# wei-zeng98/piano-a2s

Measured on AMD Instinct MI355X. Metric: training clips/sec (12 s, 5-bar), higher is better.
Workload: dtype f32

## Files before the change

### include/a2s.h

```cpp
#ifndef A2S_H
#define A2S_H
#include <stddef.h>
#include <stdint.h>
#ifdef __cplusplus
extern "C" {
#endif

#define A2S_OK 0
#define A2S_ERR_ARG (-1)
#define A2S_ERR_HIP (-2)
#define A2S_ERR_WORKSPACE (-3)

const char* a2s_last_error(void);
int a2s_version(void);
long long a2s_launch_count(void);

int a2s_gemm_f32(void* stream, int M, int N, int K, float alpha, const float* A, long sAm, long sAk,
                 const float* B, long sBk, long sBn, float beta, float* C, long ldc, const float* bias, int act,
                 int batch, long bsA, long bsB, long bsC, int splitk, float* workspace, size_t workspace_bytes);
int a2s_gemm_f32_affine(void* stream, int M, int N, int K, float alpha, const float* A, long sAm, long sAk, const float* B, long sBk,
                        long sBn, float beta, float* C, long ldc, const float* bias, int act, int batch, long bsA, long bsB, long bsC,
                        int splitk, float* workspace, size_t workspace_bytes, const float* a_scale, const float* a_shift, int a_period,
                        const float* b_scale, const float* b_shift, int b_period);
int a2s_gemm_f32_bnstats(void* stream, int M, int N, int K, const float* A, long sAm, long sAk, const float* B, long sBk, long sBn, float* C, long ldc,
                         const float* y, const float* mean, const float* invstd, const float* scale, const float* shift, int period, float* partial);
int a2s_gemm_f32_affine_scaled(void* stream, int M, int N, int K, float alpha, const float* A, long sAm, long sAk, const float* B, long sBk,
                               long sBn, float beta, float* C, long ldc, const float* bias, int act, int batch, long bsA, long bsB, long bsC,
                               int splitk, float* workspace, size_t workspace_bytes, const float* a_scale, const float* a_shift, int a_period,
                               const float* b_scale, const float* b_shift, int b_period, const float* a_absmax, const float* b_absmax);
int a2s_gemm_f32_bnstats_scaled(void* stream, int M, int N, int K, const float* A, long sAm, long sAk, const float* B, long sBk, long sBn, float* C, long ldc,
                                const float* y, const float* mean, const float* invstd, const float* scale, const float* shift, int period, float* partial,
                                const float* a_absmax, const float* b_absmax);
int a2s_linear_dgrad_bnstats(void* stream, int M, int N, int K, const float* dz, long lda, const float* Wt, float* da, long ldc, const float* y,
                             const float* mean, const float* invstd, const float* scale, const float* shift, int period, float* partial,
                             const float* dz_absmax, const float* w_absmax, float* workspace, size_t workspace_bytes, float* da_absmax_out);
int a2s_linear_fwd(void* stream, int M, int N, int K, const float* y, long lda, const float* W, float* z, long ldc, const float* scale, const float* shift,
                   int period, const float* y_absmax, const float* w_absmax, float* workspace, size_t workspace_bytes);
int a2s_linear_fwd_eligible(int M, int N, int K, int period);
int a2s_linear_wgrad(void* stream, int M, int N, int K, const float* dz, long ldz, const float* y, long lda, float* G, long ldg, const float* scale,
                     const float* shift, int period, const float* dz_absmax, const float* y_absmax, float* workspace, size_t workspace_bytes);
size_t a2s_linear_wgrad_ws_bytes(int M, int K);
int a2s_linear_wgrad_eligible(int M, int N, int K, int period);
int a2s_tallk_wgrad(void* stream, int M, int Np, int K, const float* P, long ldp, const float* A, long lda, float* G, long ldg, int transposed, float* bias,
                    const float* p_absmax, const float* a_absmax, float* workspace, size_t workspace_bytes);
size_t a2s_tallk_wgrad_ws_bytes(int M, int Np, int K);
int a2s_tallk_wgrad_eligible(int M, int Np, int K, long ldp, long lda, long ldg, int transposed);
size_t a2s_linear_dgrad_ws_bytes(int N, int K);
int a2s_linear_dgrad_blocks(int M);
int a2s_linear_dgrad_eligible(int M, int N, int K, int period);
int a2s_absmax(void* stream, const float* x, long n, float* out);
int a2s_gemm_bnstats_blocks(int M, int period);
size_t a2s_gemm_workspace_bytes(int M, int N, int batch, int splitk);
int a2s_gemm_pick_splitk(int M, int N, int K, int batch);
void a2s_gemm_debug_tile(int cfg);
int a2s_debug_set(const char* key, int value);
int a2s_debug_get(const char* key);
int a2s_env_check(void);
int a2s_persist_abort_latch(void* device_word);

int a2s_conv3x3(void* stream, const float* x, const float* w, float* y, const float* in_scale, const float* in_shift,
                float* stat_partial, int B, int T, int F, int Cin, int Cout, int flip, float* workspace);
int a2s_conv3x3_ranged(void* stream, const float* x, const float* w, float* y, const float* in_scale, const float* in_shift, const float* in_absmax,
                       float* stat_partial, float* out_absmax, int B, int T, int F, int Cin, int Cout, float* workspace);
int a2s_conv3x3_stat_blocks(int B, int T, int F, int Cin);
int a2s_conv3x3_dgrad_bnstats(void* stream, const float* dy, const float* w, float* g, const float* yl, const float* yl_mean, const float* yl_invstd,
                              const float* yl_scale, const float* yl_shift, float* stat_partial, int B, int T, int F, int Cin, int Cout,
                              float* workspace);
int a2s_bn_bwd_from_partial(void* stream, const float* g, const float* x, const float* mean, const float* invstd, const float* scale, const float* shift,
                            float* dgamma, float* dbeta, float* dx , const float* partial, int nblocks, float* c12, long rows, int C, int F);
int a2s_conv3x3_dgrad_bnstats_scaled(void* stream, const float* dy, const float* w, float* g, const float* yl, const float* yl_mean, const float* yl_invstd,
                                     const float* yl_scale, const float* yl_shift, float* stat_partial, int B, int T, int F, int Cin, int Cout,
                                     float* workspace, const float* dy_absmax);
int a2s_conv3x3_dgrad_bnstats_ranged(void* stream, const float* dy, const float* w, float* g, const float* yl, const float* yl_mean, const float* yl_invstd,
                                     const float* yl_scale, const float* yl_shift, float* stat_partial, int B, int T, int F, int Cin, int Cout,
                                     float* workspace, const float* dy_absmax, float* g_absmax_out);
int a2s_bn_bwd_from_partial_amax(void* stream, const float* g, const float* x, const float* mean, const float* invstd, const float* scale, const float* shift,
                                 float* dgamma, float* dbeta, float* dx, const float* partial, int nblocks, float* c12, long rows, int C, int F,
                                 float* dx_absmax);
size_t a2s_conv3x3_workspace_floats(int Cin);
int a2s_bn_finalize(void* stream, const float* partial, int nblocks, int C, double count, const float* gamma,
                    const float* beta, float* running_mean, float* running_var, long long* num_batches_tracked,
                    float* mean, float* invstd, float* scale, float* shift, float eps, float momentum, int training);
int a2s_bn_relu_apply(void* stream, const float* x, float* y, const float* scale, const float* shift, long n, int C, int F);
int a2s_col_stats(void* stream, const float* x, float* partial, long rows, int C, int rows_per_block);
int a2s_bn1d_relu_dropout(void* stream, const float* x, float* y, const float* scale, const float* shift,
                          const uint8_t* keep_mask, float inv_keep, long n, int C);

int a2s_gru_gates_fwd(void* stream, const float* gi, long ldgi, const float* gh, long ldgh, const float* hprev, long ldhp,
                      float* hout, long ldho, float* hout2, long ldho2, float* save, int R, int H);
int a2s_gru_seq_fwd(void* stream, const float* gi_all, long gi_bstride, long gi_tstride, const float* w_hh,
                    const float* b_hh, float* out, long out_bstride, long out_tstride, float* hbuf, float* gh,
                    float* save, float* hn, int B, int T, int H, int reverse, float* workspace, size_t workspace_bytes);

int a2s_attn_step_fwd(void* stream, const float* keys, const float* enc, const float* q, long ldq, const float* v,
                      float* ctx, long ldctx, float* ctx2, long ldctx2, float* attw, int B, int T, int H,
                      const int* n_done, int n_rows_total, float* workspace);
int a2s_attn_step_fwd_rows(void* stream, const float* keys, const float* enc, const float* q, long ldq, const float* v, float* ctx,
                           long ldctx, float* ctx2, long ldctx2, float* attw, int R, int T, int H, float* workspace, int n_clips,
                           const int* clip_order, const int* clip_rank, const int* row_until, int n_active, int step);
size_t a2s_attn_workspace_floats(int B, int T, int H);
size_t a2s_attn_workspace_floats_fused(int n_clips, int T, int H, int groups);

int a2s_log_softmax_rows(void* stream, const float* x, long ldx, float* y, long ldy, int* argmax_out, int R, int V);
int a2s_embed_rows(void* stream, const float* table, const long long* ids64, const int* ids32, long id_stride,
                   int const_id, float* out, long ldo, int col0, int R, int E, const uint8_t* keep_mask, float inv_keep);

typedef struct a2s_note_dec_args {
    const float* attn_w; const float* attn_b; const float* attn_v;
    const float* w_ih; const float* w_hh; const float* b_ih; const float* b_hh;
    const float* out_w; const float* out_b; const float* emb;
    const float* keys; const float* enc;
    float* h; float* x; float* q; float* gates; float* attw; float* o;
    float* gh; float* gi; float* logits;
    float* probs; long probs_bstride;
    const long long* gt; long gt_bstride;
    const uint8_t* tf_flags;
    const uint8_t* drop; float inv_keep;
    int* argmax_out; long am_bstride;
    int* eos_seen; long long* lengths; int* n_done;
    int* steps_exec;
    float* attn_ws;
    float* gemm_ws; size_t gemm_ws_bytes;
    int* t_base;
    const int* clip_order;
    const int* clip_rank;
    const int* row_until;
    const int* n_active;
    int n_clips;
    const int* m_active;
    const int* row_list;
    const int* n_rows_active;
    int R, T, H, E, V, steps, poll, eos_id;
    int use_graph;
    float* step_ws; size_t step_ws_floats;
    const int* tf_flags_dev;
    float* persist_ws; size_t persist_ws_bytes;
} a2s_note_dec_args;
int a2s_note_decoder_fwd(void* stream, const a2s_note_dec_args* args, int* steps_done);
int a2s_grammar_argmax_rows(void* stream, const float* x, long ldx, float* y, long ldy, const signed char* next_state, int n_states, int* row_state,
                            int* choice_out, int R, int V);
int a2s_note_decoder_fwd_grammar(void* stream, const a2s_note_dec_args* args, const signed char* next_state, int n_states, int* row_state, int* steps_done);
int a2s_grammar_launches(void);
#define A2S_BEAM_MAX 4
typedef struct a2s_beam_args {
    int K; float alpha;
    const signed char* next_state; int n_states;
    int pad_id;
    int* row_state;
    float* score; int* finished;
    int* done_count;
    int* token_hist; int* parent_hist; float* score_hist;
    float* probs_scratch;
    int* ids_out; long long* lengths_out; float* score_out;
} a2s_beam_args;
int a2s_note_decoder_fwd_beam(void* stream, const a2s_note_dec_args* args, const a2s_beam_args* beam, int* steps_done);
int a2s_beam_step(void* stream, const a2s_beam_args* beam, const float* logits, long ldl, const float* emb, float* xnext, long ldx, float* h, int h_cols,
                  float* q, int q_cols, int* n_done, int* steps_exec, int B, int V, int E, int t, int max_steps, int eos_id);
int a2s_beam_backtrack(void* stream, const a2s_beam_args* beam, float* probs, long probs_bstride, const int* steps_exec, int B, int V, int max_steps, int eos_id);
int a2s_beam_launches(void);
typedef struct a2s_align_args {
    float* attw_step;
    int* peak; float* weight; float* centroid;
    long out_stride;
    const signed char* next_state; int n_states;
    int* row_state;
} a2s_align_args;
int a2s_attn_align_rows(void* stream, const float* attw, long ldw, int R, int T, int* peak_out, float* weight_out, float* centroid_out, long out_stride);
int a2s_note_decoder_fwd_align(void* stream, const a2s_note_dec_args* args, const a2s_align_args* align, int* steps_done);
int a2s_align_launches(void);

int a2s_render_notes(void* stream, const int* programs, int rows_per_clip, int n_samples, float* wave, long wave_bstride, int B);
int a2s_render_launches(void);

int a2s_transpose_targets(void* stream, const int* new_key, const int* interval, const int* token_map, int n_rows, int V, const int* semitones,
                          const float* detune, long long* key, long long* upper, long long* lower, int bars, int U, int L, int bins_per_semitone,
                          float* eff_bins, int* counters, int B);
int a2s_shift_bins(void* stream, const float* x, float* y, const float* eff_bins, int B, int rows, int F);
int a2s_augment_launches(void);

int a2s_tempo_plan(void* stream, const float* x, int B, int rows, int F, const float* u, float R, int min_frames, int* content, int* step,
                   int* counters);
int a2s_stretch_frames(void* stream, const float* x, float* y, const int* step, int B, int rows, int F);
int a2s_tempo_launches(void);

int a2s_specaug_plan(void* stream, const float* x, int B, int rows, int F, const float* table, const unsigned* draws, int Wt, int Wf, int m,
                     int* content, int* plan, float* stats, int* counters);
int a2s_specaug_apply(void* stream, const float* x, float* y, const float* table, const int* content, const int* plan, const float* stats, int B,
                      int rows, int F);
int a2s_specaug_launches(void);

int a2s_room_ir(void* stream, const unsigned* room_seed, const int* params, int B, float* ir, long ir_bstride, int L_max);
int a2s_fir_rows(void* stream, const float* x, long x_bstride, const float* ir, long ir_bstride, const int* params, float* y, long y_bstride, int B,
                 int n_samples, int L_max);
int a2s_fir_tile_samples(void);
int a2s_fir_tap_chunk(void);
int a2s_room_launches(void);

int a2s_resample_rows(void* stream, const float* x, long x_bstride, const int* n_in, int n_in_max, int C, const float* table, int L, int M, int K, int Hh,
                      float* y, long y_bstride, int n_out_max, int B);
int a2s_resample_tile_samples(void);
int a2s_resample_launches(void);

// ... 141 lines not shown
```

### piano_a2s_amd/conv_bwd_plan.py

```python
from collections import namedtuple

CHANS = ((1, 20), (20, 20), (20, 40), (40, 40))
LIN_WGRAD_PLACES = ("before", "beside", 4, 3, 2)


class ConvBwdFlags(namedtuple("ConvBwdFlags", "fuse_bn_rows dgrad_bnstats sync_fused fuse_bn_apply fuse_bn_apply_l1 lin_wgrad_at",
                              defaults=(True, True, True, False, True, "before"))):
    """The switches of engine_bwd (module attributes there, read once per call), with their defaults.
    fuse_bn_rows: BatchNorm-backward apply inside the row-streaming weight gradient's staging waves (A2S_FUSE_BN_ROWS=0: a tensor pass of its own).
    dgrad_bnstats: the statistics of the layer below in the epilogue of the data gradient (the Linear's included).
    sync_fused: synchronised BatchNorm keeps these fused paths (one small all-reduce per layer); False: separate statistics + apply passes.
    fuse_bn_apply / fuse_bn_apply_l1: the apply inside the TILED weight gradient a2s_conv3x3_wgrad_bn (dy = scale (g' - c1 - xhat c2) formed while the
    kernel stages its dy operand), for every layer (parity-tested, slower: the extra operand pushes conv3x3_wgrad<40> from 202 to 281 registers) / for
    conv1, whose weight gradient is a kernel of its own and whose input gradient nothing else reads (one pass over (g, y) instead of two).
    lin_wgrad_at: where the Linear's weight gradient (reads y4 once, 10-11 ms, only the optimizer waits for it) is issued: "before" the data gradient on
    the main stream; "beside" it on the weight-gradient stream; 4 / 3 / 2: on that stream at the top of that layer's turn.  Step time in that order:
    454.6, 454.5, 456.9, 456.3, 463.3 ms (profiles/r06_ab_switches.txt, r06_ab_lin_wgrad_placement.txt): no placement of this launch moves the step;
    the simplest is the default."""


class LinearPlan(namedtuple("LinearPlan", "stats absmax_after dgrad wgrad_at join_side")):
    """stats: statistics source of the BatchNorm1d above the Linear (always the full form: "own" / "sync_own"); absmax_after: max |dz| by a pass of its own
    (the synchronised apply does not reduce it).  dgrad: "own" (csrc/a2s_linear.hip: partials and max |da|), "generic" (two-term GEMM tiles with the
    statistics epilogue: partials) or "gemm" (neither).  wgrad_at: see ConvBwdFlags.lin_wgrad_at; join_side: the weight gradient ran on the
    weight-gradient stream, so the main stream waits for that stream at the end of the ConvStack backward."""


class LayerPlan(namedtuple("LayerPlan", "i ci co dy_range form stats absmax_after lin_wgrad dgrad dgrad_range out_range")):
    """Layer i with channels ci -> co.
    dy_range: the layer owns a device scalar max |dy|, zeroed by the executor and reduced by the kernel that writes dy: the two-term fp16 kernels that read dy scale
    it by the matching power of two (gradients would otherwise sit in fp16's subnormal range).
    form: how BatchNorm backward and weight gradient are launched.
      "rows"  -- statistics only, then a2s_conv3x3_wgrad_bn_ranged: dy = scale (g' - c1 - xhat c2) is formed by the STAGING waves of the row-streaming
                 kernel (they wait 40-57 % of their time for the multiply waves) and written once, over g in place (every element is read and written
                 by the same thread), with its range: one pass over (g, y) less than "apply".  Needs partials and a range with the incoming gradient.
      "apply" -- the full BatchNorm backward over g in place, which writes the range (absmax_after: the synchronised one does not; a2s_absmax does),
                 then a2s_conv3x3_wgrad_ranged.
      "tiled" -- statistics only, then a2s_conv3x3_wgrad_bn, which forms dy while it stages its operand and writes it to a fresh tensor; no range.
                 Layer 1 has no data gradient, so its dy is never written: one pass over (g, y) instead of apply (read 2, write 1) + read 1.
    stats: see stats_source.  lin_wgrad: the Linear's weight gradient is issued on the weight-gradient stream before anything of this layer.
    dgrad: "bnstats" (a2s_conv3x3_dgrad_bnstats_ranged: partials for the layer below in its epilogue; dgrad_range: it is given the layer's max |dy|;
    out_range: it writes the per-channel range of what it produces), "plain" (a2s_conv3x3, flip = 1: nothing for the layer below) or "none" (layer 1)."""


def stats_source(sync_bn, stats_only, has_partial):
    if has_partial and not sync_bn:
        return "partial"
    if has_partial and stats_only:
        return "sync_partial"
    if sync_bn and stats_only:
        raise ValueError("synchronised BatchNorm backward, statistics only, without the producer's partials: not a plan")
    return "sync_own" if sync_bn else "own"


def plan_convstack_bwd(flags, sync_bn, rows, F, linear_kernels, linear_dgrad_eligible, ranged_eligible):
    if isinstance(flags.lin_wgrad_at, bool) or flags.lin_wgrad_at not in LIN_WGRAD_PLACES:
        raise ValueError(f"lin_wgrad_at = {flags.lin_wgrad_at!r}: expected one of {LIN_WGRAD_PLACES}")
    fused_ok = not sync_bn or flags.sync_fused
    stats = flags.dgrad_bnstats and fused_ok
    epilogue = stats and F >= 128 and F % 4 == 0 and rows > 64
    dgrad = ("own" if linear_kernels and linear_dgrad_eligible else "generic") if epilogue else "gemm"
    linear = LinearPlan(stats_source(sync_bn, False, False), sync_bn, dgrad, flags.lin_wgrad_at, flags.lin_wgrad_at != "before")
    partial, amax = dgrad != "gemm", dgrad == "own"
    layers = []
    for i in (4, 3, 2, 1):
        ci, co = CHANS[i - 1]
        eligible = ranged_eligible[(ci, co)] if isinstance(ranged_eligible, dict) and i > 1 else ranged_eligible
        rows_form = flags.fuse_bn_rows and fused_ok and i > 1 and partial and amax and eligible
        tiled = not sync_bn and (flags.fuse_bn_apply or (i == 1 and flags.fuse_bn_apply_l1))
        form = "rows" if rows_form else "tiled" if tiled else "apply"
        dy_range = i > 1 and fused_ok
        out_range = i > 2 and stats and flags.fuse_bn_rows
        layers.append(LayerPlan(i, ci, co, dy_range, form, stats_source(sync_bn, form != "apply", partial), form == "apply" and sync_bn and dy_range,
                                flags.lin_wgrad_at == i, "none" if i == 1 else "bnstats" if stats else "plain",
                                i > 1 and stats and dy_range and not flags.fuse_bn_apply, out_range))
        partial, amax = stats, out_range
    return linear, tuple(layers)
```

### piano_a2s_amd/csrc/a2s_api.hip

```cpp
#define A2S_SWITCHES_IMPL
#include "a2s_internal.h"

thread_local char a2s_err_msg[512] = {0};
long long a2s_launch_counter = 0;

#define ST ((hipStream_t)stream)

extern "C" {

const char* a2s_last_error(void) { return a2s_err_msg; }
int a2s_version(void) { return 1; }
long long a2s_launch_count(void) { return __atomic_load_n(&a2s_launch_counter, __ATOMIC_RELAXED); }

int a2s_gemm_f32(void* stream, int M, int N, int K, float alpha, const float* A, long sAm, long sAk, const float* B, long sBk,
                 long sBn, float beta, float* C, long ldc, const float* bias, int act, int batch, long bsA, long bsB, long bsC,
                 int splitk, float* workspace, size_t workspace_bytes) {
    return a2s_gemm_impl(ST, M, N, K, alpha, A, sAm, sAk, B, sBk, sBn, beta, C, ldc, bias, act, batch, bsA, bsB, bsC, splitk,
                         workspace, workspace_bytes);
}
int a2s_gemm_f32_affine(void* stream, int M, int N, int K, float alpha, const float* A, long sAm, long sAk, const float* B, long sBk,
                        long sBn, float beta, float* C, long ldc, const float* bias, int act, int batch, long bsA, long bsB, long bsC,
                        int splitk, float* workspace, size_t workspace_bytes, const float* a_scale, const float* a_shift, int a_period,
                        const float* b_scale, const float* b_shift, int b_period) {
    return a2s_gemm_affine_impl(ST, M, N, K, alpha, A, sAm, sAk, B, sBk, sBn, beta, C, ldc, bias, act, batch, bsA, bsB, bsC, splitk,
                                workspace, workspace_bytes, a_scale, a_shift, a_period, b_scale, b_shift, b_period,
                                nullptr, nullptr, nullptr, nullptr, nullptr, nullptr, 0, 0, nullptr, nullptr);
}
int a2s_gemm_f32_affine_scaled(void* stream, int M, int N, int K, float alpha, const float* A, long sAm, long sAk, const float* B, long sBk,
                               long sBn, float beta, float* C, long ldc, const float* bias, int act, int batch, long bsA, long bsB, long bsC,
                               int splitk, float* workspace, size_t workspace_bytes, const float* a_scale, const float* a_shift, int a_period,
                               const float* b_scale, const float* b_shift, int b_period, const float* a_absmax, const float* b_absmax) {
    return a2s_gemm_affine_impl(ST, M, N, K, alpha, A, sAm, sAk, B, sBk, sBn, beta, C, ldc, bias, act, batch, bsA, bsB, bsC, splitk,
                                workspace, workspace_bytes, a_scale, a_shift, a_period, b_scale, b_shift, b_period,
                                nullptr, nullptr, nullptr, nullptr, nullptr, nullptr, 0, 1, a_absmax, b_absmax);
}
int a2s_gemm_f32_bnstats_scaled(void* stream, int M, int N, int K, const float* A, long sAm, long sAk, const float* B, long sBk, long sBn, float* C, long ldc,
                                const float* y, const float* mean, const float* invstd, const float* scale, const float* shift, int period, float* partial,
                                const float* a_absmax, const float* b_absmax) {
    return a2s_gemm_affine_impl(ST, M, N, K, 1.f, A, sAm, sAk, B, sBk, sBn, 0.f, C, ldc, nullptr, 0, 1, 0, 0, 0, 1, nullptr, 0,
                                nullptr, nullptr, 0, nullptr, nullptr, 0, y, mean, invstd, scale, shift, partial, period, 1, a_absmax, b_absmax);
}
int a2s_absmax(void* stream, const float* x, long n, float* out) { return a2s_absmax_impl(ST, x, n, out); }
int a2s_linear_dgrad_bnstats(void* stream, int M, int N, int K, const float* dz, long lda, const float* Wt, float* da, long ldc, const float* y,
                             const float* mean, const float* invstd, const float* scale, const float* shift, int period, float* partial,
                             const float* dz_absmax, const float* w_absmax, float* workspace, size_t workspace_bytes, float* da_absmax_out) {
    return a2s_linear_dgrad_bnstats_impl(ST, M, N, K, dz, lda, Wt, 1, K, da, ldc, y, mean, invstd, scale, shift, period, partial, dz_absmax, w_absmax,
                                         workspace, workspace_bytes, da_absmax_out);
}
size_t a2s_linear_dgrad_ws_bytes(int N, int K) { return a2s_linear_dgrad_ws_bytes_impl(N, K); }
int a2s_linear_fwd(void* stream, int M, int N, int K, const float* y, long lda, const float* W, float* z, long ldc, const float* scale, const float* shift,
                   int period, const float* y_absmax, const float* w_absmax, float* workspace, size_t workspace_bytes) {
    return a2s_linear_fwd_impl(ST, M, N, K, y, lda, W, z, ldc, scale, shift, period, y_absmax, w_absmax, workspace, workspace_bytes);
}
int a2s_linear_wgrad(void* stream, int M, int N, int K, const float* dz, long ldz, const float* y, long lda, float* G, long ldg, const float* scale,
                     const float* shift, int period, const float* dz_absmax, const float* y_absmax, float* workspace, size_t workspace_bytes) {
    return a2s_linear_wgrad_impl(ST, M, N, K, dz, ldz, y, lda, G, ldg, scale, shift, period, dz_absmax, y_absmax, workspace, workspace_bytes);
}
size_t a2s_linear_wgrad_ws_bytes(int M, int K) { return a2s_linear_wgrad_ws_bytes_impl(M, K); }
int a2s_linear_wgrad_eligible(int M, int N, int K, int period) { return a2s_linear_wgrad_ok(M, N, K, 256, 4, 4, period, nullptr, nullptr, nullptr) ? 1 : 0; }
int a2s_tallk_wgrad(void* stream, int M, int Np, int K, const float* P, long ldp, const float* A, long lda, float* G, long ldg, int transposed, float* bias,
                    const float* p_absmax, const float* a_absmax, float* workspace, size_t workspace_bytes) {
    return a2s_tallk_wgrad_impl(ST, M, Np, K, P, ldp, A, lda, G, ldg, transposed, bias, p_absmax, a_absmax, workspace, workspace_bytes);
}
size_t a2s_tallk_wgrad_ws_bytes(int M, int Np, int K) { return a2s_tallk_wgrad_ws_bytes_impl(M, Np, K); }
int a2s_tallk_wgrad_eligible(int M, int Np, int K, long ldp, long lda, long ldg, int transposed) {
    return a2s_tallk_wgrad_ok(M, Np, K, ldp, lda, ldg, transposed, nullptr, nullptr, nullptr, nullptr) ? 1 : 0;
}
int a2s_linear_fwd_eligible(int M, int N, int K, int period) { return a2s_linear_fwd_ok(M, N, K, 4, 4, period, nullptr, nullptr, nullptr) ? 1 : 0; }
int a2s_linear_dgrad_blocks(int M) { return a2s_linear_dgrad_blocks_impl(M); }
int a2s_linear_dgrad_eligible(int M, int N, int K, int period) {
    return a2s_linear_dgrad_ok(M, N, K, 4, 1, K, 4, period, nullptr, nullptr, nullptr, nullptr) ? 1 : 0;
}
int a2s_gemm_f32_bnstats(void* stream, int M, int N, int K, const float* A, long sAm, long sAk, const float* B, long sBk, long sBn, float* C, long ldc,
                         const float* y, const float* mean, const float* invstd, const float* scale, const float* shift, int period, float* partial) {
    return a2s_gemm_affine_impl(ST, M, N, K, 1.f, A, sAm, sAk, B, sBk, sBn, 0.f, C, ldc, nullptr, 0, 1, 0, 0, 0, 1, nullptr, 0,
                                nullptr, nullptr, 0, nullptr, nullptr, 0, y, mean, invstd, scale, shift, partial, period, 0, nullptr, nullptr);
}
int a2s_gemm_bnstats_blocks(int M, int period) { return a2s_cdiv(M, 128) * a2s_gemm_bnstats_slots(period); }
size_t a2s_gemm_workspace_bytes(int M, int N, int batch, int splitk) { return a2s_gemm_workspace_bytes_impl(M, N, batch, splitk); }
int a2s_gemm_pick_splitk(int M, int N, int K, int batch) { return a2s_gemm_pick_splitk_impl(M, N, K, batch); }
void a2s_gemm_debug_tile(int cfg) { a2s_gemm_debug_tile_impl(cfg); }
size_t a2s_note_step_workspace_floats(int H, int E) { return a2s_note_step_workspace_floats_impl(H, E); }
int a2s_debug_set(const char* key, int value) {
    if (!key) return A2S_ERR_ARG;
    const int id = a2s_switch_find(key);
    if (id >= 0) { a2s_switch_store(id, value); return A2S_OK; }
    if (!strcmp(key, "attn_deferred_fast")) { a2s_attn_deferred_fast = value ? 1 : 0; return A2S_OK; }
    if (!strcmp(key, "tallk_wgrad")) { a2s_tallk_wgrad_on = value ? 1 : 0; return A2S_OK; }
    if (!strcmp(key, "tallk_wgrad_max_splits")) { a2s_tallk_wgrad_max_splits = value > 0 ? value : 0; return A2S_OK; }
    if (!strcmp(key, "gemm_tile")) { a2s_gemm_debug_tile_impl(value); return A2S_OK; }
    snprintf(a2s_err_msg, sizeof(a2s_err_msg), "a2s_debug_set: unknown key %s", key);
    return A2S_ERR_ARG;
}
int a2s_env_check(void) {
    if (const char* e = a2s_switch_env_error()) A2S_FAIL(A2S_ERR_ARG, "%s: expected a decimal number >= 0", e);
    return A2S_OK;
}

int a2s_persist_abort_latch(void* device_word) { a2s_persist_latch_set(device_word); return A2S_OK; }

int a2s_debug_get(const char* key) {
    if (!key) return -1;
    const int id = a2s_switch_find(key);
    if (id == A2S_SW_attn_pair_fused_rows) return a2s_attn_pair_fused_rows();
    if (id >= 0) return a2s_sw((a2s_switch)id);
    if (!strcmp(key, "attn_pair_launches")) return (int)a2s_attn_pair_launches();
    if (!strcmp(key, "attn_pair_bwd_launches")) return (int)a2s_attn_pair_bwd_launches();
    if (!strcmp(key, "attn_deferred_fast")) return a2s_attn_deferred_fast;
    if (!strcmp(key, "tallk_wgrad")) return a2s_tallk_wgrad_on;
    if (!strcmp(key, "tallk_wgrad_max_splits")) return a2s_tallk_wgrad_max_splits;
    if (!strcmp(key, "tallk_wgrad_launches")) return (int)a2s_tallk_wgrad_launches();
    if (!strcmp(key, "attn_dk_ahead_launches")) return (int)a2s_attn_dk_ahead_launches();
    if (!strcmp(key, "attn_denc_launches")) return (int)a2s_attn_denc_launches();
    if (!strcmp(key, "dec_mid_launches")) return a2s_dec_mid_launches();
    if (!strcmp(key, "dec_persist_launches")) return a2s_dec_persist_launches();
    if (!strcmp(key, "edit_distance_launches")) return (int)a2s_edit_distance_launches();
    if (!strcmp(key, "conv_rows16_c20_launches")) return (int)a2s_conv_rows16_c20_launches();
    if (!strcmp(key, "device_cus")) return a2s_device_geometry().cus;
    if (!strcmp(key, "device_xccs")) return a2s_device_geometry().xccs;
    return -1;
}

int a2s_conv3x3(void* stream, const float* x, const float* w, float* y, const float* in_scale, const float* in_shift,
                float* stat_partial, int B, int T, int F, int Cin, int Cout, int flip, float* workspace) {
    return a2s_conv3x3_impl(ST, x, w, y, in_scale, in_shift, stat_partial, B, T, F, Cin, Cout, flip, workspace, nullptr, nullptr, nullptr, nullptr, nullptr, nullptr,
                            nullptr, nullptr);
}
int a2s_conv3x3_ranged(void* stream, const float* x, const float* w, float* y, const float* in_scale, const float* in_shift, const float* in_absmax,
                       float* stat_partial, float* out_absmax, int B, int T, int F, int Cin, int Cout, float* workspace) {
    return a2s_conv3x3_impl(ST, x, w, y, in_scale, in_shift, stat_partial, B, T, F, Cin, Cout, 0, workspace, nullptr, nullptr, nullptr, nullptr, nullptr, nullptr,
                            in_absmax, out_absmax);
}
int a2s_conv3x3_dgrad_bnstats(void* stream, const float* dy, const float* w, float* g, const float* yl, const float* yl_mean, const float* yl_invstd,
                              const float* yl_scale, const float* yl_shift, float* stat_partial, int B, int T, int F, int Cin, int Cout,
                              float* workspace) {
    if (!yl) { snprintf(a2s_err_msg, sizeof(a2s_err_msg), "conv3x3_dgrad_bnstats: yl is required"); return A2S_ERR_ARG; }
    return a2s_conv3x3_impl(ST, dy, w, g, nullptr, nullptr, stat_partial, B, T, F, Cin, Cout, 1, workspace, yl, yl_mean, yl_invstd, yl_scale, yl_shift, nullptr, nullptr, nullptr);
}
int a2s_conv3x3_dgrad_bnstats_scaled(void* stream, const float* dy, const float* w, float* g, const float* yl, const float* yl_mean, const float* yl_invstd,
                                     const float* yl_scale, const float* yl_shift, float* stat_partial, int B, int T, int F, int Cin, int Cout,
                                     float* workspace, const float* dy_absmax) {
    if (!yl) { snprintf(a2s_err_msg, sizeof(a2s_err_msg), "conv3x3_dgrad_bnstats_scaled: yl is required"); return A2S_ERR_ARG; }
    return a2s_conv3x3_impl(ST, dy, w, g, nullptr, nullptr, stat_partial, B, T, F, Cin, Cout, 1, workspace, yl, yl_mean, yl_invstd, yl_scale, yl_shift, dy_absmax, nullptr, nullptr);
}
int a2s_conv3x3_dgrad_bnstats_ranged(void* stream, const float* dy, const float* w, float* g, const float* yl, const float* yl_mean, const float* yl_invstd,
                                     const float* yl_scale, const float* yl_shift, float* stat_partial, int B, int T, int F, int Cin, int Cout,
                                     float* workspace, const float* dy_absmax, float* g_absmax_out) {
    if (!yl) { snprintf(a2s_err_msg, sizeof(a2s_err_msg), "conv3x3_dgrad_bnstats_ranged: yl is required"); return A2S_ERR_ARG; }
    return a2s_conv3x3_impl(ST, dy, w, g, nullptr, nullptr, stat_partial, B, T, F, Cin, Cout, 1, workspace, yl, yl_mean, yl_invstd, yl_scale, yl_shift, dy_absmax, nullptr, g_absmax_out);
}
int a2s_bn_bwd_from_partial(void* stream, const float* g, const float* x, const float* mean, const float* invstd, const float* scale, const float* shift,
                            float* dgamma, float* dbeta, float* dx, const float* partial, int nblocks, float* c12, long rows, int C, int F) {
    return a2s_bn_bwd_from_partial_impl(ST, g, x, mean, invstd, scale, shift, dgamma, dbeta, dx, partial, nblocks, c12, rows, C, F, nullptr);
}
int a2s_bn_bwd_from_partial_amax(void* stream, const float* g, const float* x, const float* mean, const float* invstd, const float* scale, const float* shift,
                                 float* dgamma, float* dbeta, float* dx, const float* partial, int nblocks, float* c12, long rows, int C, int F,
                                 float* dx_absmax) {
    return a2s_bn_bwd_from_partial_impl(ST, g, x, mean, invstd, scale, shift, dgamma, dbeta, dx, partial, nblocks, c12, rows, C, F, dx_absmax);
}
size_t a2s_conv3x3_workspace_floats(int Cin) { return a2s_conv3x3_workspace_floats_impl(Cin); }
int a2s_conv3x3_stat_blocks(int B, int T, int F, int Cin) { return a2s_conv3x3_stat_blocks_impl(B, T, F, Cin); }
int a2s_bn_finalize(void* stream, const float* partial, int nblocks, int C, double count, const float* gamma, const float* beta,
                    float* running_mean, float* running_var, long long* nbt, float* mean, float* invstd, float* scale,
                    float* shift, float eps, float momentum, int training) {
    return a2s_bn_finalize_impl(ST, partial, nblocks, C, count, gamma, beta, running_mean, running_var, nbt, mean, invstd, scale,
                                shift, eps, momentum, training);
}
int a2s_bn_relu_apply(void* stream, const float* x, float* y, const float* scale, const float* shift, long n, int C, int F) {
    return a2s_bn_relu_apply_impl(ST, x, y, scale, shift, n, C, F);
}
int a2s_col_stats(void* stream, const float* x, float* partial, long rows, int C, int rows_per_block) {
    return a2s_col_stats_impl(ST, x, partial, rows, C, rows_per_block);
}
int a2s_bn1d_relu_dropout(void* stream, const float* x, float* y, const float* scale, const float* shift, const uint8_t* keep_mask,
                          float inv_keep, long n, int C) {
    return a2s_bn1d_relu_dropout_impl(ST, x, y, scale, shift, keep_mask, inv_keep, n, C);
}
int a2s_gru_gates_fwd(void* stream, const float* gi, long ldgi, const float* gh, long ldgh, const float* hprev, long ldhp,
                      float* hout, long ldho, float* hout2, long ldho2, float* save, int R, int H) {
    return a2s_gru_gates_fwd_impl(ST, gi, ldgi, gh, ldgh, hprev, ldhp, hout, ldho, hout2, ldho2, save, R, H);
}
int a2s_gru_seq_fwd(void* stream, const float* gi_all, long gi_bstride, long gi_tstride, const float* w_hh, const float* b_hh,
                    float* out, long out_bstride, long out_tstride, float* hbuf, float* gh, float* save, float* hn, int B, int T,
                    int H, int reverse, float* workspace, size_t workspace_bytes) {
    return a2s_gru_seq_fwd_impl(ST, gi_all, gi_bstride, gi_tstride, w_hh, b_hh, out, out_bstride, out_tstride, hbuf, gh, save, hn,
                                B, T, H, reverse, workspace, workspace_bytes);
}
int a2s_attn_step_fwd(void* stream, const float* keys, const float* enc, const float* q, long ldq, const float* v, float* ctx,
                      long ldctx, float* ctx2, long ldctx2, float* attw, int B, int T, int H, const int* n_done, int n_rows_total, float* workspace) {
    return a2s_attn_step_fwd_impl(ST, keys, enc, q, ldq, v, ctx, ldctx, ctx2, ldctx2, attw, B, T, H, n_done, n_rows_total, workspace, nullptr);
}
int a2s_attn_step_fwd_rows(void* stream, const float* keys, const float* enc, const float* q, long ldq, const float* v, float* ctx,
                           long ldctx, float* ctx2, long ldctx2, float* attw, int R, int T, int H, float* workspace, int n_clips,
                           const int* clip_order, const int* clip_rank, const int* row_until, int n_active, int step) {
    a2s_attn_rows rows = {clip_order, clip_rank, row_until, n_clips, n_active, step};
    return a2s_attn_step_fwd_impl(ST, keys, enc, q, ldq, v, ctx, ldctx, ctx2, ldctx2, attw, R, T, H, nullptr, 0, workspace, &rows);
}
size_t a2s_attn_workspace_floats(int B, int T, int H) { return a2s_attn_workspace_floats_impl(B, T, H, 1); }
size_t a2s_attn_workspace_floats_fused(int n_clips, int T, int H, int groups) { return a2s_attn_workspace_floats_impl(n_clips, T, H, groups); }
int a2s_log_softmax_rows(void* stream, const float* x, long ldx, float* y, long ldy, int* argmax_out, int R, int V) {
    return a2s_log_softmax_rows_impl(ST, x, ldx, y, ldy, argmax_out, R, V);
}
int a2s_embed_rows(void* stream, const float* table, const long long* ids64, const int* ids32, long id_stride, int const_id,
                   float* out, long ldo, int col0, int R, int E, const uint8_t* keep_mask, float inv_keep) {
    return a2s_embed_rows_impl(ST, table, ids64, ids32, id_stride, const_id, out, ldo, col0, R, E, keep_mask, inv_keep);
}
int a2s_note_decoder_fwd(void* stream, const a2s_note_dec_args* args, int* steps_done) {
    if (!args) { snprintf(a2s_err_msg, sizeof(a2s_err_msg), "note_decoder_fwd: null args"); return A2S_ERR_ARG; }
    return a2s_note_decoder_fwd_impl(ST, *args, steps_done);
}
int a2s_grammar_argmax_rows(void* stream, const float* x, long ldx, float* y, long ldy, const signed char* next_state, int n_states, int* row_state,
                            int* choice_out, int R, int V) {
    return a2s_grammar_argmax_rows_impl(ST, x, ldx, y, ldy, next_state, n_states, row_state, choice_out, R, V);
}
int a2s_note_decoder_fwd_grammar(void* stream, const a2s_note_dec_args* args, const signed char* next_state, int n_states, int* row_state, int* steps_done) {
    if (!args) { snprintf(a2s_err_msg, sizeof(a2s_err_msg), "note_decoder_fwd_grammar: null args"); return A2S_ERR_ARG; }
    const a2s_grammar_ref g = {next_state, n_states, row_state};
    return a2s_note_decoder_fwd_grammar_impl(ST, *args, g, steps_done);
}
int a2s_grammar_launches(void) { return a2s_grammar_launches_impl(); }
int a2s_note_decoder_fwd_beam(void* stream, const a2s_note_dec_args* args, const a2s_beam_args* beam, int* steps_done) {
    if (!args || !beam) { snprintf(a2s_err_msg, sizeof(a2s_err_msg), "note_decoder_fwd_beam: null args"); return A2S_ERR_ARG; }
    return a2s_note_decoder_fwd_beam_impl(ST, *args, *beam, steps_done);
}
int a2s_beam_step(void* stream, const a2s_beam_args* beam, const float* logits, long ldl, const float* emb, float* xnext, long ldx, float* h, int h_cols,
                  float* q, int q_cols, int* n_done, int* steps_exec, int B, int V, int E, int t, int max_steps, int eos_id) {
    if (!beam) { snprintf(a2s_err_msg, sizeof(a2s_err_msg), "beam_step: null args"); return A2S_ERR_ARG; }
    const a2s_beam_args& g = *beam;
    const BeamStepArgs a = {logits, ldl, emb, xnext, ldx, h, h_cols, q, q_cols, g.next_state, g.n_states, g.row_state, g.score, g.finished, g.done_count,
                            g.token_hist, g.parent_hist, g.score_hist, g.probs_scratch, n_done, steps_exec, B, g.K, V, E, t, max_steps, eos_id, g.pad_id};
    return a2s_beam_step_finalize_impl(ST, a);
}
int a2s_beam_backtrack(void* stream, const a2s_beam_args* beam, float* probs, long probs_bstride, const int* steps_exec, int B, int V, int max_steps, int eos_id) {
    if (!beam) { snprintf(a2s_err_msg, sizeof(a2s_err_msg), "beam_backtrack: null args"); return A2S_ERR_ARG; }
    const a2s_beam_args& g = *beam;
    const BeamBackArgs a = {g.score, g.token_hist, g.parent_hist, g.probs_scratch, probs, probs_bstride, g.ids_out, (long)max_steps, g.lengths_out, g.score_out,
                            steps_exec, g.alpha, B, g.K, V, max_steps, eos_id, g.pad_id};
    return a2s_beam_backtrack_impl(ST, a);
}
int a2s_beam_launches(void) { return a2s_beam_launches_impl(); }
int a2s_attn_align_rows(void* stream, const float* attw, long ldw, int R, int T, int* peak_out, float* weight_out, float* centroid_out, long out_stride) {
    return a2s_attn_align_rows_impl(ST, attw, ldw, R, T, peak_out, weight_out, centroid_out, out_stride);
}
int a2s_note_decoder_fwd_align(void* stream, const a2s_note_dec_args* args, const a2s_align_args* align, int* steps_done) {
    if (!args || !align) { snprintf(a2s_err_msg, sizeof(a2s_err_msg), "note_decoder_fwd_align: null args"); return A2S_ERR_ARG; }
    return a2s_note_decoder_fwd_align_impl(ST, *args, *align, steps_done);
}
int a2s_align_launches(void) { return a2s_align_launches_impl(); }
int a2s_render_notes(void* stream, const int* programs, int rows_per_clip, int n_samples, float* wave, long wave_bstride, int B) {
    return a2s_render_notes_impl(ST, programs, rows_per_clip, n_samples, wave, wave_bstride, B);
}
int a2s_render_launches(void) { return a2s_render_launches_impl(); }
int a2s_transpose_targets(void* stream, const int* new_key, const int* interval, const int* token_map, int n_rows, int V, const int* semitones,
                          const float* detune, long long* key, long long* upper, long long* lower, int bars, int U, int L, int bins_per_semitone,
                          float* eff_bins, int* counters, int B) {
    return a2s_transpose_targets_impl(ST, new_key, interval, token_map, n_rows, V, semitones, detune, key, upper, lower, bars, U, L, bins_per_semitone, eff_bins,
                                      counters, B);
}
int a2s_shift_bins(void* stream, const float* x, float* y, const float* eff_bins, int B, int rows, int F) {
    return a2s_shift_bins_impl(ST, x, y, eff_bins, B, rows, F);
}
int a2s_augment_launches(void) { return a2s_augment_launches_impl(); }
// ... 228 lines not shown
```

### piano_a2s_amd/csrc/a2s_internal.h

```cpp
#pragma once
#include "a2s_common.h"
#include "../../include/a2s.h"
#include "a2s_switches.h"

static inline int a2s_attn_pair_fused_rows(void) {
    const int cap = a2s_sw(A2S_SW_dec_fused_max_rows), v = a2s_sw(A2S_SW_attn_pair_fused_rows);
    return v < cap ? v : cap;
}
static inline unsigned a2s_persist_dbg(void) {
    return (a2s_sw(A2S_SW_persist_force_agent) ? PERSIST_DBG_FORCE_AGENT : 0u) | (a2s_sw(A2S_SW_persist_inject_abort) ? PERSIST_DBG_INJECT_ABORT : 0u);
}

int a2s_absmax_impl(hipStream_t st, const float* x, long n, float* out);
size_t a2s_gemm_workspace_bytes_impl(int M, int N, int batch, int splitk);
int a2s_gemm_pick_splitk_impl(int M, int N, int K, int batch);
int a2s_gemm_bnstats_slots(int period);
void a2s_gemm_debug_tile_impl(int cfg);
int a2s_gemm_affine_impl(hipStream_t st, int M, int N, int K, float alpha, const float* A, long sAm, long sAk,
    const float* B, long sBk, long sBn, float beta, float* C, long ldc, const float* bias, int act,
    int batch, long bsA, long bsB, long bsC, int splitk, float* ws, size_t ws_bytes,
    const float* a_scale, const float* a_shift, int a_period, const float* b_scale, const float* b_shift, int b_period,
    const float* ep_y, const float* ep_mean, const float* ep_invstd, const float* ep_scale, const float* ep_shift,
    float* ep_partial, int ep_period, int two_term, const float* a_absmax, const float* b_absmax);
int a2s_gemm_impl(hipStream_t st, int M, int N, int K, float alpha, const float* A, long sAm, long sAk,
    const float* B, long sBk, long sBn, float beta, float* C, long ldc, const float* bias, int act,
    int batch, long bsA, long bsB, long bsC, int splitk, float* ws, size_t ws_bytes);

size_t a2s_linear_dgrad_ws_bytes_impl(int N, int K);
int a2s_linear_dgrad_blocks_impl(int M);
bool a2s_linear_dgrad_ok(int M, int N, int K, long lda, long sBk, long sBn, long ldc, int period, const void* A, const void* B, const void* C, const void* y);
int a2s_linear_dgrad_bnstats_impl(hipStream_t st, int M, int N, int K, const float* A, long lda, const float* Wt, long sBk, long sBn, float* C, long ldc,
    const float* ep_y, const float* mean, const float* invstd, const float* scale, const float* shift, int period,
    float* partial, const float* a_absmax, const float* b_absmax, float* ws, size_t ws_bytes, float* c_absmax_out);
bool a2s_linear_fwd_ok(int M, int N, int K, long lda, long ldc, int period, const void* A, const void* W, const void* C);
int a2s_linear_fwd_impl(hipStream_t st, int M, int N, int K, const float* A, long lda, const float* W, float* C, long ldc, const float* a_scale,
    const float* a_shift, int period, const float* a_absmax, const float* w_absmax, float* ws, size_t ws_bytes);
size_t a2s_linear_wgrad_ws_bytes_impl(int M, int K);
bool a2s_linear_wgrad_ok(int M, int N, int K, long ldz, long lda, long ldg, int period, const void* dz, const void* A, const void* G);
int a2s_linear_wgrad_impl(hipStream_t st, int M, int N, int K, const float* dz, long ldz, const float* A, long lda, float* G, long ldg, const float* a_scale,
    const float* a_shift, int period, const float* dz_absmax, const float* a_absmax, float* ws, size_t ws_bytes);
extern int a2s_tallk_wgrad_on;
extern int a2s_tallk_wgrad_max_splits;
long a2s_tallk_wgrad_launches(void);
size_t a2s_tallk_wgrad_ws_bytes_impl(int M, int Np, int K);
bool a2s_tallk_wgrad_ok(int M, int Np, int K, long ldp, long lda, long ldg, int transposed, const void* P, const void* A, const void* G, const void* bias);
int a2s_tallk_wgrad_impl(hipStream_t st, int M, int Np, int K, const float* P, long ldp, const float* A, long lda, float* G, long ldg, int transposed,
    float* bias, const float* p_absmax, const float* a_absmax, float* ws, size_t ws_bytes);

int a2s_act_bound_impl(hipStream_t st, const float* scale, const float* shift, const float* absmax, int C, float* out);
size_t a2s_conv3x3_workspace_floats_impl(int Cin);
int a2s_conv3x3_impl(hipStream_t st, const float* x, const float* w, float* y, const float* in_scale,
    const float* in_shift, float* stat_partial, int B, int T, int F, int Cin, int Cout, int flip, float* ws,
    const float* yl, const float* yl_mean, const float* yl_invstd, const float* yl_scale, const float* yl_shift,
    const float* x_absmax, const float* in_absmax, float* out_absmax);
int a2s_conv3x3_stat_blocks_impl(int B, int T, int F, int Cin);
int a2s_bn_finalize_impl(hipStream_t st, const float* partial, int nblocks, int C, double count, const float* gamma,
    const float* beta, float* running_mean, float* running_var, long long* nbt, float* mean,
    float* invstd, float* scale, float* shift, float eps, float momentum, int training);
int a2s_bn_relu_apply_impl(hipStream_t st, const float* x, float* y, const float* scale, const float* shift, long n, int C, int F);
int a2s_col_stats_impl(hipStream_t st, const float* x, float* partial, long rows, int C, int rows_per_block);
int a2s_bn1d_relu_dropout_impl(hipStream_t st, const float* x, float* y, const float* scale, const float* shift,
    const uint8_t* mask, float inv_keep, long n, int C);
size_t a2s_conv3x3_wgrad_workspace_bytes_impl(int Cin, int Cout);
int a2s_conv3x3_wgrad_impl(hipStream_t st, const float* dy, const float* x, const float* in_scale, const float* in_shift, float* dW,
    float* ws, size_t ws_bytes, int B, int T, int F, int Cin, int Cout, const float* bn_y, const float* bn_mean,
    const float* bn_invstd, const float* bn_scale, const float* bn_shift, const float* bn_c12, float* dy_out,
    const float* dy_absmax, const float* act_absmax);
int a2s_bn_bwd_impl(hipStream_t st, const float* g, const float* x, const float* mean, const float* invstd, const float* scale,
    const float* shift, const uint8_t* mask, float inv_keep, float* dgamma, float* dbeta, float* dx, float* partial,
    float* c12, long rows, int C, int F, float* dx_absmax);
int a2s_bn_bwd_from_partial_impl(hipStream_t st, const float* g, const float* x, const float* mean, const float* invstd, const float* scale,
    const float* shift, float* dgamma, float* dbeta, float* dx, const float* partial, int nblocks, float* c12,
    long rows, int C, int F, float* dx_absmax);
int a2s_bn_bwd_stats_impl(hipStream_t st, const float* g, const float* x, const float* mean, const float* invstd, const float* scale,
    const float* shift, const uint8_t* mask, float inv_keep, float* partial, float* sums, long rows, int C, int F);
int a2s_bn_bwd_apply_impl(hipStream_t st, const float* g, const float* x, const float* mean, const float* invstd, const float* scale,
    const float* shift, const uint8_t* mask, float inv_keep, const float* sums_local, const float* sums_global,
    double count_global, float* dgamma, float* dbeta, float* dx, float* c12, long rows, int C, int F);
int a2s_bn_bwd_sums_from_partial_impl(hipStream_t st, const float* partial, int nblocks, int C, float* sums);
int a2s_bn_bwd_c12_from_sums_impl(hipStream_t st, const float* sums_local, const float* sums_global, double count_global, float* dgamma, float* dbeta,
    float* c12, int C);
size_t a2s_bn_bwd_partial_floats_impl(long rows, int C, int F);

int a2s_channel_absmax_impl(hipStream_t st, const float* x, long rows, int C, int F, float* out);
bool a2s_conv_rows_eligible(int F, int Cin);
int a2s_conv_rows_blocks(int B, int T, int F);
size_t a2s_conv_rows_workspace_floats(int Cin);
long a2s_conv_rows16_c20_launches(void);
int a2s_conv3x3_rows_impl(hipStream_t st, const float* x, const float* w, float* y, const float* in_scale, const float* in_shift,
    const float* in_absmax, float* stat_partial, float* out_absmax, int B, int T, int F, int Cin, int Cout, int flip,
    float* ws, const float* yl, const float* yl_mean, const float* yl_invstd, const float* yl_scale, const float* yl_shift,
    const float* x_absmax);

bool a2s_wgrad_rows_eligible(int F, int Cin, int Cout);
int a2s_conv3x3_wgrad_rows_bn_impl(hipStream_t st, const float* g, const float* y, const float* mean, const float* invstd, const float* scale,
    const float* shift, const float* c12, const float* g_absmax, int g_absmax_n, const float* y_absmax, float* dz_out,
    float* dz_absmax_out, const float* x, const float* in_scale, const float* in_shift, float* dW, float* ws, size_t ws_bytes,
    int B, int T, int F, int Cin, int Cout, const float* act_absmax);
int a2s_conv3x3_wgrad_rows_impl(hipStream_t st, const float* dy, const float* x, const float* in_scale, const float* in_shift, float* dW, float* ws,
    size_t ws_bytes, int B, int T, int F, int Cin, int Cout, const float* dy_absmax, const float* act_absmax);

struct StepFinArgs {
    const float* logits; long ldl;
    float* probs; long probs_bstride;
    const long long* gt; long gt_bstride;
    const float* emb;
    float* xnext; long ldx;
    const uint8_t* drop; float inv_keep;
    int* argmax_out; long am_bstride;
    int* eos_seen; long long* lengths; int* n_done; int* steps_exec;
    const int* t_base;
    const int* row_until;
    int n_clips;
    int R, V, E, t, teacher_force, eos_id, max_t;
};
struct a2s_grammar_ref { const signed char* next; int n_states; int* row_state; };
int a2s_gru_gates_fwd_impl(hipStream_t st, const float* gi, long ldgi, const float* gh, long ldgh, const float* hprev,
    long ldhp, float* hout, long ldho, float* hout2, long ldho2, float* save, int R, int H);
int a2s_gru_bptt_step_impl(hipStream_t st, const float* dgh, const float* w_hh_t, const float* dhz_in, const float* dout, long ld_dout,
    const float* save, const float* hprev, long ld_hprev, float* dgi, long ld_dgi, float* dgh_out, float* dgh2,
    long ld_dgh2, float* dhz_out, int R, int H);
int a2s_skinny_gemm_acc_impl(hipStream_t st, const float* A, long lda, const float* Bt, long ldb, float* Cm, long ldc, int R, int N, int K);
int a2s_gru_seq_fwd_impl(hipStream_t st, const float* gi_all, long gi_bstride, long gi_tstride, const float* w_hh,
    const float* b_hh, float* out, long out_bstride, long out_tstride, float* hbuf, float* gh,
    float* save, float* hn, int B, int T, int H, int reverse, float* ws, size_t ws_bytes);
int a2s_attn_step_fwd_impl(hipStream_t st, const float* Kmat, const float* enc, const float* q, long ldq, const float* v,
    float* ctx, long ldctx, float* ctx2, long ldctx2, float* attw, int B, int T, int H,
    const int* n_done, int n_rows_total, float* ws, const a2s_attn_rows* rows = nullptr, a2s_attn_deferred* defer = nullptr);
int a2s_log_softmax_rows_impl(hipStream_t st, const float* x, long ldx, float* y, long ldy, int* argmax_out, int R, int V);
int a2s_embed_rows_impl(hipStream_t st, const float* table, const long long* ids64, const int* ids32, long id_stride,
    int const_id, float* out, long ldo, int col0, int R, int E, const uint8_t* drop, float inv_keep);
int a2s_note_decoder_fwd_impl(hipStream_t st, const a2s_note_dec_args& a, int* steps_done);
int a2s_note_decoder_fwd_grammar_impl(hipStream_t st, const a2s_note_dec_args& a, const a2s_grammar_ref& g, int* steps_done);
int a2s_note_decoder_fwd_pair_impl(hipStream_t su, hipStream_t sl, const a2s_note_dec_args& au, const a2s_note_dec_args& al, const int* pair_order,
    const int* pair_rank, const int* pair_n_active, int* done_u, int* done_l);
int a2s_staff_emb_fwd_impl(hipStream_t st, const float* note_emb, const float* const* w ,
    const long long* ids64, const int* ids32, long id_bstride, const long long* lengths,
    long len_stride, float* out, long ldo, int col0, float* hsave, int R, int maxlen, int E, int S);
int a2s_note_decoder_zero_unwritten(hipStream_t st, const a2s_note_dec_args& a, const char* who );
size_t a2s_attn_workspace_floats_impl(int B, int T, int H, int groups);
size_t a2s_attn_bulk_lds(size_t shm, int n_active, int backward);
long a2s_attn_pair_launches(void);
struct AttnPairStep { const int* clip_order; const int* clip_rank; int n_clips; int n_active; int step; int G; int chunk; };
int a2s_pair_events(const char* who, hipEvent_t** ev_out);
static inline int a2s_record_wait(hipEvent_t ev, hipStream_t from, hipStream_t to, const char* who) {
    hipError_t e = hipEventRecord(ev, from);
    if (e == hipSuccess) e = hipStreamWaitEvent(to, ev, 0);
    if (e != hipSuccess) A2S_FAIL(A2S_ERR_HIP, "%s: event: %s", who, hipGetErrorString(e));
    return A2S_OK;
}

int a2s_log_softmax_bwd_rows_impl(hipStream_t st, const float* g, const float* y, long outer_stride, int inner, float* dx,
    int R, int V, int n_outer, int time_major);
int a2s_gru_gates_bwd_impl(hipStream_t st, const float* dh_a, long lda, const float* dh_b, long ldb, const float* save,
    const float* hprev, long ldhp, float* dgi, long ldgi, float* dgh, long ldgh, float* dgh2, long ldgh2,
    float* dhprev, long lddp, int R, int H);
int a2s_attn_step_bwd_impl(hipStream_t st, const float* Kmat, const float* enc, const float* q, long ldq, const float* v,
    const float* attw, const float* ctx, long ldctx, const float* dctx_a, long ldda, const float* dctx_b,
    long lddb, float* dctx_out, long lddo, float* dq, long lddq, float* ds_out, int B, int T, int H, float* ws,
    const a2s_attn_rows* rows = nullptr);
int a2s_attn_dk_accum_impl(hipStream_t st, const float* Kmat, const float* q_all, const float* ds_all, const float* v,
    float* dK, float* dv_partial, int B, int T, int S, int H, const int* row_until, int groups);
int a2s_attn_denc_accum_impl(hipStream_t st, const float* attw_all, const float* dctx_all, float* dEnc, int B, int T, int S, int H2,
    const int* row_until, int groups);
long a2s_attn_dk_ahead_launches(void);
long a2s_attn_denc_launches(void);
int a2s_col_sum_impl(hipStream_t st, const float* x, long ld, float* out, long rows, int C, float alpha, float beta, float* ws, size_t ws_floats);
int a2s_embed_scatter_add_impl(hipStream_t st, float* table_grad, const long long* ids64, const int* ids32, long id_stride,
    int const_id, const float* g, long ldg, int col0, int R, int E, const uint8_t* drop, float inv_keep);
int a2s_ew_act_bwd_impl(hipStream_t st, const float* g, const float* y, float* dx, long n, int act);
int a2s_note_decoder_bwd_impl(hipStream_t st, const a2s_note_dec_bwd_args& a);
int a2s_note_decoder_bwd_pair_impl(hipStream_t su, hipStream_t sl, const a2s_note_dec_bwd_args& au, const a2s_note_dec_bwd_args& al, const int* pair_order,
    const int* pair_rank, const int* pair_n_active);
int a2s_gru_seq_bwd_impl(hipStream_t st, const float* dout, long do_bstride, long do_tstride, const float* out, long out_bstride,
    long out_tstride, const float* gates, const float* w_hh, const float* dhn, float* dgi_all, float* dgh_shift,
    float* dgh_first, float* dhbuf, float* dgh_tmp, int B, int T, int H, int reverse, float* ws, size_t ws_bytes,
    float* ranges_out, int* ranges_valid);
int a2s_staff_emb_bwd_impl(hipStream_t st, const float* note_emb, const float* const* w, float* const* grads_dev, float* note_emb_grad,
    const long long* ids64, const int* ids32, long id_bstride, const long long* lengths, long len_stride,
    const float* dout, long lddo, int col0, const float* hsave, int R, int maxlen, int E, int S);
long a2s_attn_pair_bwd_launches(void);

size_t a2s_note_step_fused_head_floats(void);
size_t a2s_note_step_workspace_floats_impl(int H, int E);
int a2s_dec_mid_launches(void);
bool a2s_dec_step_fusable(int R, int H, int E, int V, const void* const* ptrs, int nptrs, const float* ws, size_t ws_floats, bool greedy = false);
int a2s_note_step_fused_fwd(hipStream_t st, const a2s_note_dec_args& a, int si, int so, int sv, int sv_next, int t, const int* t_base, int tf, bool last,
    int nrows, const int* rowmap, const a2s_attn_deferred* defer = nullptr);
int a2s_note_step_fused_bwd_prepare(hipStream_t st, const a2s_note_dec_bwd_args& a);
int a2s_note_step_fused_bwd(hipStream_t st, const a2s_note_dec_bwd_args& a, int s, const float* dh_in, float* dh_out, const a2s_attn_rows* rows,
    int nrows, const int* rowmap);
bool a2s_note_step_mid_ok(int H, int E, const void* const* ptrs, int nptrs);
int a2s_note_step_mid_gru(hipStream_t st, const a2s_note_dec_args& a, int si, int so, int sv, int sv_next, int nrows, const int* rowmap);
// ... 163 lines not shown
```

### piano_a2s_amd/csrc/a2s_linear.hip

```cpp
#include "a2s_internal.h"

#define LIN_BM 128
#define LIN_K 256
#define LIN_RS 288
#define LIN_NTH 512
#define LIN_LDS (2 * 2 * LIN_BM * LIN_RS)

typedef unsigned lu32x4 __attribute__((ext_vector_type(4)));

struct LinDgradArgs {
    const float* A; long lda;
    const unsigned char* planes;
    float* C; long ldc;
    const float* ep_y;
    const float* mean; const float* invstd; const float* scale; const float* shift;
    float* partial;
    const float* a_absmax; const float* b_absmax;
    int M, N, period, channels;
    float* c_absmax_out;
};

__global__ __launch_bounds__(256) void lin_pack_planes_k(const float* __restrict__ W, long ld, int N, int K, const float* __restrict__ absmax,
                                                         unsigned char* __restrict__ out) {
    const long id = (long)blockIdx.x * 256 + threadIdx.x;
    const int kgroups = K >> 3, nks = K >> 5;
    const int n = (int)(id / kgroups), kg = (int)(id % kgroups);
    if (n >= N) return;
    const float ps = ldexpf(1.f, pow2_scale_exp(*absmax, 12));
    const f32x4 v0 = *reinterpret_cast<const f32x4*>(W + (long)n * ld + kg * 8);
    const f32x4 v1 = *reinterpret_cast<const f32x4*>(W + (long)n * ld + kg * 8 + 4);
    float x[8];
#pragma unroll
    for (int i = 0; i < 4; ++i) { x[i] = __builtin_amdgcn_fmed3f(v0[i] * ps, -65000.f, 65000.f); x[4 + i] = __builtin_amdgcn_fmed3f(v1[i] * ps, -65000.f, 65000.f); }
    lu32x4 hi, lo;
#pragma unroll
    for (int i = 0; i < 4; ++i) { unsigned h, l; split2_pair_f16(x[2 * i], x[2 * i + 1], h, l); hi[i] = h; lo[i] = l; }
    const int nt = n >> 4, lr = n & 15, ks = kg >> 2, lk = kg & 3;
    unsigned char* o = out + ((((long)nt * nks + ks) * 2) * 64 + (lk * 16 + lr)) * 16;
    *reinterpret_cast<lu32x4*>(o) = hi;
    *reinterpret_cast<lu32x4*>(o + 64 * 16) = lo;
}

__global__ __launch_bounds__(LIN_NTH) void lin_dgrad_bnstats(LinDgradArgs a) {
    __shared__ __attribute__((aligned(16))) unsigned char lds[LIN_LDS];
    const int tid = threadIdx.x, lane = tid & 63, wave = tid >> 6, lr = lane & 15, lk = lane >> 4;
    const int m0 = blockIdx.x * LIN_BM;
    const int ka = pow2_scale_exp(*a.a_absmax, 12), kb = pow2_scale_exp(*a.b_absmax, 12);
    const float psa = ldexpf(1.f, ka), unscale = ldexpf(1.f, -(ka + kb));

    {
        f32x4 v[16];
#pragma unroll
        for (int i = 0; i < 16; ++i) {
            const int slot = tid + LIN_NTH * i, row = slot >> 6, k = (slot & 63) * 4;
            v[i] = (f32x4){0.f, 0.f, 0.f, 0.f};
            if (m0 + row < a.M) v[i] = *reinterpret_cast<const f32x4*>(a.A + (long)(m0 + row) * a.lda + k);
        }
#pragma unroll
        for (int i = 0; i < 16; ++i) {
            const int slot = tid + LIN_NTH * i, row = slot >> 6, k = (slot & 63) * 4;
            float x[4];
#pragma unroll
            for (int j = 0; j < 4; ++j) x[j] = __builtin_amdgcn_fmed3f(v[i][j] * psa, -65000.f, 65000.f);
            uint2 hi, lo;
            split2_pair_f16(x[0], x[1], hi.x, lo.x);
            split2_pair_f16(x[2], x[3], hi.y, lo.y);
            const int blk = k >> 7, off = (k & 127) * 2;
            *reinterpret_cast<uint2*>(lds + ((blk * 2 + 0) * LIN_BM + row) * LIN_RS + off) = hi;
            *reinterpret_cast<uint2*>(lds + ((blk * 2 + 1) * LIN_BM + row) * LIN_RS + off) = lo;
        }
    }
    __syncthreads();

    const int ntiles = (a.N + 255) >> 8;
    const unsigned lane_off = (unsigned)(lr * a.ldc + lk * 4) * 4u;
    float s1 = 0.f, s2 = 0.f, vmax = 0.f;
    int cur_c = -1;
    auto flush = [&]() {
        if (cur_c < 0) return;
        const float w1 = wave_sum(s1), w2 = wave_sum(s2);
        if (lane == 0) {
            float* p = a.partial + (((long)blockIdx.x * 8 + wave) * a.channels + cur_c) * 2;
            p[0] = w1; p[1] = w2;
        }
    };
    lu32x4 bf[3][2][2];
    auto load_b = [&](int n0, int ks, lu32x4 (&dst)[2][2]) {
        const unsigned char* bp = a.planes + (long)(n0 >> 4) * 8 * 2 * 64 * 16;
#pragma unroll
        for (int nt = 0; nt < 2; ++nt)
#pragma unroll
            for (int sp = 0; sp < 2; ++sp) dst[nt][sp] = *reinterpret_cast<const lu32x4*>(bp + ((long)(nt * 8 + ks) * 2 + sp) * 1024 + (unsigned)lane * 16u);
    };
    if (wave * 32 < a.N) { load_b(wave * 32, 0, bf[0]); load_b(wave * 32, 1, bf[1]); }
    for (int j = 0; j < ntiles; ++j) {
        const int n0 = j * 256 + wave * 32;
        if (n0 >= a.N) break;
        f32x4 yq[8][2];
        auto load_y = [&](int mt) {
            const int m = m0 + mt * 16 + lr;
#pragma unroll
            for (int nt = 0; nt < 2; ++nt) {
#if defined(LIN_X) && LIN_X >= 1 && LIN_X != 4
                yq[mt][nt] = (f32x4){1.f, 1.f, 1.f, 1.f};
#else
                yq[mt][nt] = (f32x4){0.f, 0.f, 0.f, 0.f};
                if (m < a.M)
                    yq[mt][nt] = *reinterpret_cast<const f32x4*>(reinterpret_cast<const char*>(a.ep_y + (long)(m0 + mt * 16) * a.ldc + n0 + nt * 16) + lane_off);
#endif
            }
        };
#pragma unroll
        for (int mt = 0; mt < 3; ++mt) load_y(mt);
        f32x4 acc[8][2];
#pragma unroll
        for (int mt = 0; mt < 8; ++mt)
#pragma unroll
            for (int nt = 0; nt < 2; ++nt) acc[mt][nt] = (f32x4){0.f, 0.f, 0.f, 0.f};
#pragma unroll
        for (int ks = 0; ks < 8; ++ks) {
#if defined(LIN_X) && LIN_X >= 3
            if (ks + 2 < 8 && a.M < 0) load_b(n0, ks + 2, bf[(ks + 2) % 3]);
#else
            if (ks + 2 < 8) load_b(n0, ks + 2, bf[(ks + 2) % 3]);
#endif
#pragma unroll
            for (int half = 0; half < 2; ++half) {
                lu32x4 af[2][4];
#pragma unroll
                for (int sp = 0; sp < 2; ++sp)
#pragma unroll
                    for (int q = 0; q < 4; ++q)
                        af[sp][q] = *reinterpret_cast<const lu32x4*>(lds + (((ks >> 2) * 2 + sp) * LIN_BM + (half * 4 + q) * 16 + lr) * LIN_RS + (ks & 3) * 64 + lk * 16);
#define LIN_PRODUCT(SA, SB)                                                                                                   \
                _Pragma("unroll") for (int nt = 0; nt < 2; ++nt)                                                              \
                    _Pragma("unroll") for (int q = 0; q < 4; ++q)                                                             \
                        acc[half * 4 + q][nt] = __builtin_amdgcn_mfma_f32_16x16x32_f16(__builtin_bit_cast(f16x8, bf[ks % 3][nt][SB]), \
                                                                                       __builtin_bit_cast(f16x8, af[SA][q]), acc[half * 4 + q][nt], 0, 0, 0);
                LIN_PRODUCT(1, 0) LIN_PRODUCT(0, 1) LIN_PRODUCT(0, 0)
#undef LIN_PRODUCT
            }
        }
        if (n0 + 256 < a.N) { load_b(n0 + 256, 0, bf[0]); load_b(n0 + 256, 1, bf[1]); }
#pragma unroll
        for (int mt = 3; mt < 8; ++mt) load_y(mt);
        const int c = n0 / a.period;
        if (c != cur_c) { flush(); s1 = 0.f; s2 = 0.f; cur_c = c; }
        const float mean = a.mean[c], invstd = a.invstd[c], sc = a.scale[c], sh = a.shift[c];
#pragma unroll
        for (int mt = 0; mt < 8; ++mt) {
            const int m = m0 + mt * 16 + lr;
            if (m >= a.M) continue;
#pragma unroll
            for (int nt = 0; nt < 2; ++nt) {
                f32x4 v = acc[mt][nt];
#pragma unroll
                for (int r = 0; r < 4; ++r) { v[r] *= unscale; vmax = fmaxf(vmax, fabsf(v[r])); }
#if defined(LIN_X) && LIN_X >= 2
                if (v[0] == 123.456f)
#endif
                *reinterpret_cast<f32x4*>(reinterpret_cast<char*>(a.C + (long)(m0 + mt * 16) * a.ldc + n0 + nt * 16) + lane_off) = v;
#pragma unroll
                for (int r = 0; r < 4; ++r) {
                    const float gm = (fmaf(yq[mt][nt][r], sc, sh) > 0.f) ? v[r] : 0.f;
                    s1 += gm; s2 = fmaf(gm * (yq[mt][nt][r] - mean), invstd, s2);
                }
            }
        }
    }
    flush();
    if (a.c_absmax_out) {
        const float m = wave_max(vmax);
        if (lane == 0 && m > 0.f) atomicMax(reinterpret_cast<unsigned*>(a.c_absmax_out), __float_as_uint(m));
    }
}

size_t a2s_linear_dgrad_ws_bytes_impl(int N, int K) { return (K > 0 && K % 32 == 0 && N > 0) ? (size_t)N * K * 2 * 2 : 0; }
int a2s_linear_dgrad_blocks_impl(int M) { return M > 0 ? ((M + LIN_BM - 1) / LIN_BM) * 8 : 0; }

bool a2s_linear_dgrad_ok(int M, int N, int K, long lda, long sBk, long sBn, long ldc, int period, const void* A, const void* B, const void* C, const void* y) {
    return K == LIN_K && M >= LIN_BM && N >= 256 && N % 32 == 0 && period > 0 && period % 32 == 0 && N % period == 0 && N / period <= 4096 && sBk == 1 && sBn == K &&
           lda % 4 == 0 && ldc % 4 == 0 && (((uintptr_t)A | (uintptr_t)B | (uintptr_t)C | (uintptr_t)y) % 16 == 0);
}

int a2s_linear_dgrad_bnstats_impl(hipStream_t st, int M, int N, int K, const float* A, long lda, const float* Wt, long sBk, long sBn, float* C, long ldc,
                                  const float* ep_y, const float* mean, const float* invstd, const float* scale, const float* shift, int period,
                                  float* partial, const float* a_absmax, const float* b_absmax, float* ws, size_t ws_bytes, float* c_absmax_out) {
    A2S_REQUIRE(A && Wt && C && ep_y && mean && invstd && scale && shift && partial && a_absmax && b_absmax && ws, "linear_dgrad_bnstats: null argument");
    A2S_REQUIRE(a2s_linear_dgrad_ok(M, N, K, lda, sBk, sBn, ldc, period, A, Wt, C, ep_y),
                "linear_dgrad_bnstats: needs K = 256, M >= 128, N >= 256, N %% 32 == 0, period %% 32 == 0, a k-contiguous weight (N x K) and 16-byte aligned rows");
    A2S_REQUIRE(((uintptr_t)ws % 16 == 0) && ws_bytes >= a2s_linear_dgrad_ws_bytes_impl(N, K), "linear_dgrad_bnstats: workspace too small (%zu bytes needed)",
                a2s_linear_dgrad_ws_bytes_impl(N, K));
    const int channels = N / period, nblk = a2s_linear_dgrad_blocks_impl(M);
    hipError_t e = hipMemsetAsync(partial, 0, sizeof(float) * 2 * (size_t)nblk * channels, st);
    if (e != hipSuccess) A2S_FAIL(A2S_ERR_HIP, "linear_dgrad_bnstats memset: %s", hipGetErrorString(e));
    unsigned char* planes = reinterpret_cast<unsigned char*>(ws);
    hipLaunchKernelGGL(lin_pack_planes_k, dim3((unsigned)(((long)N * (K / 8) + 255) / 256)), dim3(256), 0, st, Wt, (long)K, N, K, b_absmax, planes);
    A2S_CHECK_LAUNCH("lin_pack_planes_k");
    LinDgradArgs a{A, lda, planes, C, ldc, ep_y, mean, invstd, scale, shift, partial, a_absmax, b_absmax, M, N, period, channels, c_absmax_out};
    hipLaunchKernelGGL(lin_dgrad_bnstats, dim3((M + LIN_BM - 1) / LIN_BM), dim3(LIN_NTH), 0, st, a);
    A2S_CHECK_LAUNCH("lin_dgrad_bnstats");
    return A2S_OK;
}

#define LF_RS 160
#define LF_STAGE (2 * LIN_BM * LF_RS)
#define LF_NS 3

struct LinFwdArgs {
    const float* A; long lda;
    const unsigned char* planes;
    float* C; long ldc;
    const float* a_scale; const float* a_shift;
    const float* a_absmax; const float* b_absmax;
    int M, K, period;
};

__global__ __launch_bounds__(LIN_NTH) void lin_fwd_roles(LinFwdArgs a) {
    __shared__ __attribute__((aligned(16))) unsigned char lds[LF_NS * LF_STAGE];
    const int tid = threadIdx.x, lane = tid & 63, lr = lane & 15, lk = lane >> 4;
    const int wave = __builtin_amdgcn_readfirstlane(tid >> 6);
    const int m0 = blockIdx.x * LIN_BM;
    const int ka = a.a_absmax ? pow2_scale_exp(*a.a_absmax, 12) : 0, kb = pow2_scale_exp(*a.b_absmax, 12);
    const float psa = ldexpf(1.f, ka), unscale = ldexpf(1.f, -(ka + kb));
    const int nks = a.K >> 5, nblk = a.K >> 6, kpc = a.period >> 5;
    const bool affine = a.a_scale != nullptr;
    if (wave >= 4) {
        const int st_ = tid - 256;
        const int sk = (st_ & 15) * 4;
        const bool second = sk >= 32;
        f32x4 ar[2][8];
        auto issue_a = [&](int blk, f32x4 (&r)[8]) {
#pragma unroll
            for (int i = 0; i < 8; ++i) {
                const int row = (st_ + 256 * i) >> 4;
                r[i] = (f32x4){0.f, 0.f, 0.f, 0.f};
                if (m0 + row < a.M && blk < nblk) r[i] = __builtin_nontemporal_load(reinterpret_cast<const f32x4*>(a.A + (long)(m0 + row) * a.lda + (long)blk * 64 + sk));
            }
        };
        auto commit_a = [&](int blk, const f32x4 (&r)[8]) {
            if (blk >= nblk) return;
            const int c0 = (2 * blk) / kpc, c1 = (2 * blk + 1) / kpc;
            const float sc = affine ? (second ? a.a_scale[c1] : a.a_scale[c0]) * psa : psa, sh = affine ? (second ? a.a_shift[c1] : a.a_shift[c0]) * psa : 0.f;
            const float floor_ = affine ? 0.f : -INFINITY;
            unsigned char* st = lds + (blk % LF_NS) * LF_STAGE;
#pragma unroll
            for (int i = 0; i < 8; ++i) {
                const int row = (st_ + 256 * i) >> 4;
                float x[4];
#pragma unroll
                for (int j = 0; j < 4; ++j) x[j] = __builtin_amdgcn_fmed3f(fmaxf(fmaf(r[i][j], sc, sh), floor_), -65000.f, 65000.f);
                uint2 hi, lo;
                split2_pair_f16(x[0], x[1], hi.x, lo.x);
                split2_pair_f16(x[2], x[3], hi.y, lo.y);
                *reinterpret_cast<uint2*>(st + (0 * LIN_BM + row) * LF_RS + sk * 2) = hi;
                *reinterpret_cast<uint2*>(st + (1 * LIN_BM + row) * LF_RS + sk * 2) = lo;
            }
        };
        issue_a(0, ar[0]);
        commit_a(0, ar[0]);
        issue_a(1, ar[1]); issue_a(2, ar[0]);
#pragma unroll 1
        for (int b0 = 0; b0 < nblk; b0 += 2) {
            __syncthreads();
            commit_a(b0 + 1, ar[1]); issue_a(b0 + 3, ar[1]);
            if (b0 + 1 < nblk) {
                __syncthreads();
                commit_a(b0 + 2, ar[0]); issue_a(b0 + 4, ar[0]);
            }
        }
        return;
    }
    lu32x4 bf[2][4][2];
    auto load_b = [&](int ks, lu32x4 (&dst)[4][2]) {
        if (ks >= nks) return;
#pragma unroll
        for (int nt = 0; nt < 4; ++nt)
#pragma unroll
            for (int sp = 0; sp < 2; ++sp)
                dst[nt][sp] = *reinterpret_cast<const lu32x4*>(a.planes + (((long)(wave * 4 + nt) * nks + ks) * 2 + sp) * 1024 + (unsigned)lane * 16u);
    };
    f32x4 acc[8][4];
#pragma unroll
    for (int mt = 0; mt < 8; ++mt)
#pragma unroll
        for (int nt = 0; nt < 4; ++nt) acc[mt][nt] = (f32x4){0.f, 0.f, 0.f, 0.f};
    load_b(0, bf[0]);
    auto load_af = [&](const unsigned char* st, int h, int qt, lu32x4 (&af)[2][2]) {
#pragma unroll
        for (int sp = 0; sp < 2; ++sp)
#pragma unroll
            for (int q = 0; q < 2; ++q) af[sp][q] = *reinterpret_cast<const lu32x4*>(st + (sp * LIN_BM + (qt * 2 + q) * 16 + lr) * LF_RS + h * 64 + lk * 16);
    };
    auto multiply = [&](int qt, const lu32x4 (&af)[2][2], const lu32x4 (&b)[4][2]) {
#define LR_PRODUCT(SA, SB)                                                                                                        \
        _Pragma("unroll") for (int nt = 0; nt < 4; ++nt)                                                                          \
            _Pragma("unroll") for (int q = 0; q < 2; ++q)                                                                         \
                acc[qt * 2 + q][nt] = __builtin_amdgcn_mfma_f32_16x16x32_f16(__builtin_bit_cast(f16x8, b[nt][SB]),                \
                                                                             __builtin_bit_cast(f16x8, af[SA][q]), acc[qt * 2 + q][nt], 0, 0, 0);
        LR_PRODUCT(1, 0) LR_PRODUCT(0, 1) LR_PRODUCT(0, 0)
#undef LR_PRODUCT
    };
#pragma unroll 1
    for (int blk = 0; blk < nblk; ++blk) {
        __syncthreads();
        const unsigned char* st = lds + (blk % LF_NS) * LF_STAGE;
        lu32x4 fa[2][2], fb[2][2];
        load_af(st, 0, 0, fa);
        load_b(2 * blk + 1, bf[1]);
        __builtin_amdgcn_sched_barrier(0);
        load_af(st, 0, 1, fb); multiply(0, fa, bf[0]);
        __builtin_amdgcn_sched_barrier(0);
        load_af(st, 0, 2, fa); multiply(1, fb, bf[0]);
        __builtin_amdgcn_sched_barrier(0);
        load_af(st, 0, 3, fb); multiply(2, fa, bf[0]);
        __builtin_amdgcn_sched_barrier(0);
        load_af(st, 1, 0, fa); multiply(3, fb, bf[0]);
        __builtin_amdgcn_sched_barrier(0);
        load_b(2 * blk + 2, bf[0]);
        load_af(st, 1, 1, fb); multiply(0, fa, bf[1]);
        __builtin_amdgcn_sched_barrier(0);
        load_af(st, 1, 2, fa); multiply(1, fb, bf[1]);
        __builtin_amdgcn_sched_barrier(0);
        load_af(st, 1, 3, fb); multiply(2, fa, bf[1]);
        __builtin_amdgcn_sched_barrier(0);
        multiply(3, fb, bf[1]);
        __builtin_amdgcn_sched_barrier(0);
    }
#pragma unroll
    for (int mt = 0; mt < 8; ++mt) {
        const int m = m0 + mt * 16 + lr;
        if (m >= a.M) continue;
#pragma unroll
        for (int nt = 0; nt < 4; ++nt) {
            f32x4 v = acc[mt][nt];
#pragma unroll
            for (int r = 0; r < 4; ++r) v[r] *= unscale;
            *reinterpret_cast<f32x4*>(a.C + (long)m * a.ldc + wave * 64 + nt * 16 + lk * 4) = v;
        }
    }
}

bool a2s_linear_fwd_ok(int M, int N, int K, long lda, long ldc, int period, const void* A, const void* W, const void* C) {
    return N == 256 && M >= 1 && K >= 128 && K % 64 == 0 && (period == 0 || (period % 32 == 0 && K % period == 0)) && lda % 4 == 0 && ldc % 4 == 0 &&
           (((uintptr_t)A | (uintptr_t)W | (uintptr_t)C) % 16 == 0);
}

int a2s_linear_fwd_impl(hipStream_t st, int M, int N, int K, const float* A, long lda, const float* W, float* C, long ldc, const float* a_scale,
                        const float* a_shift, int period, const float* a_absmax, const float* w_absmax, float* ws, size_t ws_bytes) {
    A2S_REQUIRE(A && W && C && w_absmax && ws && ((a_scale == nullptr) == (a_shift == nullptr)), "linear_fwd: null argument");
    A2S_REQUIRE(a2s_linear_fwd_ok(M, N, K, lda, ldc, a_scale ? period : 0, A, W, C),
                "linear_fwd: needs N = 256, K %% 64 == 0, period %% 32 == 0 and 16-byte aligned rows");
    A2S_REQUIRE(((uintptr_t)ws % 16 == 0) && ws_bytes >= (size_t)N * K * 4, "linear_fwd: workspace too small (%zu bytes needed)", (size_t)N * K * 4);
    unsigned char* planes = reinterpret_cast<unsigned char*>(ws);
    hipLaunchKernelGGL(lin_pack_planes_k, dim3((unsigned)(((long)N * (K / 8) + 255) / 256)), dim3(256), 0, st, W, (long)K, N, K, w_absmax, planes);
    A2S_CHECK_LAUNCH("lin_pack_planes_k");
    LinFwdArgs a{A, lda, planes, C, ldc, a_scale, a_shift, a_absmax, w_absmax, M, K, a_scale ? period : K};
    hipLaunchKernelGGL(lin_fwd_roles, dim3((M + LIN_BM - 1) / LIN_BM), dim3(LIN_NTH), 0, st, a);
    A2S_CHECK_LAUNCH("lin_fwd");
    return A2S_OK;
}

struct LinWgradArgs {
    const float* A; long lda;
    const unsigned char* planes;
    float* partial;
    const float* a_scale; const float* a_shift;
    const float* a_absmax; const float* d_absmax;
    int M, K, period, nblk, blk_per_split;
    long plane_stride; int np;
    float* bias_partial;
};

__global__ __launch_bounds__(256) void lin_pack_dz_planes(const float* __restrict__ dz, long ld, int M, int nsteps, const float* __restrict__ absmax,
                                                          unsigned char* __restrict__ out) {
    const long id = (long)blockIdx.x * 256 + threadIdx.x;
    const int n = (int)(id & 255), lk = (int)((id >> 8) & 3), s = (int)(id >> 10);
    if (s >= nsteps) return;
    dz += blockIdx.y * 256;
    out += (size_t)blockIdx.y * nsteps * (16 * 2 * 1024);
    float ps = ldexpf(1.f, pow2_scale_exp(*absmax, 12));
    if ((s >> 3) & 1) ps = -ps;
    float x[8];
#pragma unroll
    for (int j = 0; j < 8; ++j) {
        const int m = s * 32 + lk * 8 + j;
        x[j] = m < M ? __builtin_amdgcn_fmed3f(dz[(long)m * ld + n] * ps, -65000.f, 65000.f) : 0.f;
    }
    lu32x4 hi, lo;
#pragma unroll
    for (int i = 0; i < 4; ++i) { unsigned h, l; split2_pair_f16(x[2 * i], x[2 * i + 1], h, l); hi[i] = h; lo[i] = l; }
    unsigned char* o = out + ((((long)s * 16 + (n >> 4)) * 2) * 64 + (lk * 16 + (n & 15))) * 16;
    *reinterpret_cast<lu32x4*>(o) = hi;
    *reinterpret_cast<lu32x4*>(o + 64 * 16) = lo;
}

template <bool BIAS>
__global__ __launch_bounds__(LIN_NTH) void lin_wgrad_roles(LinWgradArgs a) {
    __shared__ __attribute__((aligned(16))) unsigned char lds[LF_NS * LF_STAGE];
    const int tid = threadIdx.x, lane = tid & 63, lr = lane & 15, lk = lane >> 4;
    const int wave = __builtin_amdgcn_readfirstlane(tid >> 6);
    const int k0 = blockIdx.x * LIN_BM;
    const int b_lo = blockIdx.y * a.blk_per_split, b_hi = min(a.nblk, b_lo + a.blk_per_split);
    const int ka = a.a_absmax ? pow2_scale_exp(*a.a_absmax, 12) : 0, kd = pow2_scale_exp(*a.d_absmax, 12);
    const float psa = ldexpf(1.f, ka), unscale = ldexpf(1.f, -(ka + kd));
    const bool affine = a.a_scale != nullptr;
    if (wave >= 4) {
        const int st_ = tid - 256;
        const int rq = st_ & 15, cq0 = st_ >> 4;
        float sc[2], sh[2];
#pragma unroll
        for (int u = 0; u < 2; ++u) {
            const int ch = affine ? (k0 + 4 * (cq0 + 16 * u)) / a.period : 0;
            sc[u] = affine ? a.a_scale[ch] * psa : psa; sh[u] = affine ? a.a_shift[ch] * psa : 0.f;
        }
        const float floor_ = affine ? 0.f : -INFINITY;
        f32x4 ar[2][8];
        f32x4 bs[2] = {(f32x4){0.f, 0.f, 0.f, 0.f}, (f32x4){0.f, 0.f, 0.f, 0.f}};
        auto issue_a = [&](int blk, f32x4 (&r)[8]) {
#pragma unroll
            for (int u = 0; u < 2; ++u)
#pragma unroll
                for (int j = 0; j < 4; ++j) {
                    const int m = blk * 64 + 4 * rq + j;
                    r[4 * u + j] = (f32x4){0.f, 0.f, 0.f, 0.f};
                    if (m < a.M && blk < b_hi) r[4 * u + j] = __builtin_nontemporal_load(reinterpret_cast<const f32x4*>(a.A + (long)m * a.lda + k0 + 4 * (cq0 + 16 * u)));
                }
        };
        auto commit_a = [&](int blk, const f32x4 (&r)[8]) {
            if (blk >= b_hi) return;
            unsigned char* st = lds + (blk % LF_NS) * LF_STAGE;
            if (BIAS) {
#pragma unroll
                for (int u = 0; u < 2; ++u)
#pragma unroll
                    for (int j = 0; j < 4; ++j)
#pragma unroll
                        for (int c = 0; c < 4; ++c) bs[u][c] += r[4 * u + j][c];
            }
#pragma unroll
            for (int u = 0; u < 2; ++u)
#pragma unroll
                for (int c = 0; c < 4; ++c) {
                    float x[4];
#pragma unroll
                    for (int j = 0; j < 4; ++j) x[j] = __builtin_amdgcn_fmed3f(fmaxf(fmaf(r[4 * u + j][c], sc[u], sh[u]), floor_), -65000.f, 65000.f);
                    uint2 hi, lo;
                    split2_pair_f16(x[0], x[1], hi.x, lo.x);
                    split2_pair_f16(x[2], x[3], hi.y, lo.y);
                    *reinterpret_cast<uint2*>(st + (0 * LIN_BM + 4 * (cq0 + 16 * u) + c) * LF_RS + rq * 8) = hi;
                    *reinterpret_cast<uint2*>(st + (1 * LIN_BM + 4 * (cq0 + 16 * u) + c) * LF_RS + rq * 8) = lo;
                }
        };
        if (b_lo < b_hi) {
            issue_a(b_lo, ar[0]);
            commit_a(b_lo, ar[0]);
            issue_a(b_lo + 1, ar[1]); issue_a(b_lo + 2, ar[0]);
        }
#pragma unroll 1
        for (int b = b_lo; b < b_hi; b += 2) {
            __syncthreads();
            commit_a(b + 1, ar[1]); issue_a(b + 3, ar[1]);
            if (b + 1 < b_hi) {
                __syncthreads();
                commit_a(b + 2, ar[0]); issue_a(b + 4, ar[0]);
            }
        }
        if (BIAS && blockIdx.z == 0) {
#pragma unroll
            for (int u = 0; u < 2; ++u) {
#pragma unroll
                for (int c = 0; c < 4; ++c)
#pragma unroll
                    for (int o = 1; o < 16; o <<= 1) bs[u][c] += __shfl_xor(bs[u][c], o, 64);
                if (rq == 0) *reinterpret_cast<f32x4*>(a.bias_partial + (long)blockIdx.y * a.K + k0 + 4 * (cq0 + 16 * u)) = bs[u];
            }
        }
        return;
    }
    lu32x4 df[2][4][2];
    const unsigned char* planes = a.planes + blockIdx.z * a.plane_stride;
    auto load_d = [&](int step, lu32x4 (&dst)[4][2]) {
        if (step >= 2 * b_hi) return;
#pragma unroll
        for (int nt = 0; nt < 4; ++nt)
#pragma unroll
            for (int sp = 0; sp < 2; ++sp)
                dst[nt][sp] = *reinterpret_cast<const lu32x4*>(planes + ((((long)step) * 16 + wave * 4 + nt) * 2 + sp) * 1024 + (unsigned)lane * 16u);
    };
    f32x4 acc[8][4];
#pragma unroll
    for (int kt = 0; kt < 8; ++kt)
#pragma unroll
        for (int nt = 0; nt < 4; ++nt) acc[kt][nt] = (f32x4){0.f, 0.f, 0.f, 0.f};
    bool neg = false;
    auto flip = [&]() {
#pragma unroll
        for (int kt = 0; kt < 8; ++kt)
#pragma unroll
            for (int nt = 0; nt < 4; ++nt)
#pragma unroll
                for (int r = 0; r < 4; ++r) acc[kt][nt][r] = -acc[kt][nt][r];
    };
    auto load_bf = [&](const unsigned char* st, int h, int qt, lu32x4 (&f)[2][2]) {
#pragma unroll
        for (int sp = 0; sp < 2; ++sp)
#pragma unroll
            for (int q = 0; q < 2; ++q) f[sp][q] = *reinterpret_cast<const lu32x4*>(st + (sp * LIN_BM + (qt * 2 + q) * 16 + lr) * LF_RS + h * 64 + lk * 16);
    };
    auto multiply = [&](int qt, const lu32x4 (&f)[2][2], const lu32x4 (&d)[4][2]) {
#define LW_PRODUCT(SX, SD)                                                                                                        \
        _Pragma("unroll") for (int nt = 0; nt < 4; ++nt)                                                                          \
            _Pragma("unroll") for (int q = 0; q < 2; ++q)                                                                         \
                acc[qt * 2 + q][nt] = __builtin_amdgcn_mfma_f32_16x16x32_f16(__builtin_bit_cast(f16x8, f[SX][q]),                 \
                                                                             __builtin_bit_cast(f16x8, d[nt][SD]), acc[qt * 2 + q][nt], 0, 0, 0);
        LW_PRODUCT(1, 0) LW_PRODUCT(0, 1) LW_PRODUCT(0, 0)
#undef LW_PRODUCT
    };
    load_d(2 * b_lo, df[0]);
#pragma unroll 1
    for (int blk = b_lo; blk < b_hi; ++blk) {
        const bool want = ((2 * blk) >> 3) & 1;
        if (want != neg) { flip(); neg = want; }
        __syncthreads();
        const unsigned char* st = lds + (blk % LF_NS) * LF_STAGE;
        lu32x4 fa[2][2], fb[2][2];
        load_bf(st, 0, 0, fa);
        load_d(2 * blk + 1, df[1]);
        __builtin_amdgcn_sched_barrier(0);
        load_bf(st, 0, 1, fb); multiply(0, fa, df[0]);
        __builtin_amdgcn_sched_barrier(0);
        load_bf(st, 0, 2, fa); multiply(1, fb, df[0]);
        __builtin_amdgcn_sched_barrier(0);
        load_bf(st, 0, 3, fb); multiply(2, fa, df[0]);
        __builtin_amdgcn_sched_barrier(0);
        load_bf(st, 1, 0, fa); multiply(3, fb, df[0]);
        __builtin_amdgcn_sched_barrier(0);
        load_d(2 * blk + 2, df[0]);
        load_bf(st, 1, 1, fb); multiply(0, fa, df[1]);
        __builtin_amdgcn_sched_barrier(0);
        load_bf(st, 1, 2, fa); multiply(1, fb, df[1]);
        __builtin_amdgcn_sched_barrier(0);
        load_bf(st, 1, 3, fb); multiply(2, fa, df[1]);
        __builtin_amdgcn_sched_barrier(0);
        multiply(3, fb, df[1]);
        __builtin_amdgcn_sched_barrier(0);
    }
    if (neg) flip();
    float* slab = a.partial + ((long)blockIdx.y * a.np + blockIdx.z * 256) * a.K;
#pragma unroll
    for (int kt = 0; kt < 8; ++kt)
#pragma unroll
        for (int nt = 0; nt < 4; ++nt) {
            f32x4 v = acc[kt][nt];
#pragma unroll
            for (int r = 0; r < 4; ++r) v[r] *= unscale;
            *reinterpret_cast<f32x4*>(slab + (long)(wave * 64 + nt * 16 + lr) * a.K + k0 + kt * 16 + lk * 4) = v;
        }
}

template <bool TR>
__global__ __launch_bounds__(256) void lin_wgrad_reduce(const float* __restrict__ partial, int splits, long n, float* __restrict__ G, long ldg, int K,
                                                        const float* __restrict__ bias_partial, float* __restrict__ bias) {
    const long i = ((long)blockIdx.x * 256 + threadIdx.x) * 4;
    if (i >= n) {
        const long k = i - n;
        if (!bias_partial || k >= K) return;
        f32x4 s = *reinterpret_cast<const f32x4*>(bias_partial + k);
        for (int p = 1; p < splits; ++p) {
            const f32x4 v = *reinterpret_cast<const f32x4*>(bias_partial + (long)p * K + k);
#pragma unroll
            for (int r = 0; r < 4; ++r) s[r] += v[r];
        }
#pragma unroll
        for (int r = 0; r < 4; ++r) bias[k + r] += s[r];
        return;
    }
    f32x4 s = *reinterpret_cast<const f32x4*>(partial + i);
    for (int p = 1; p < splits; ++p) {
        const f32x4 v = *reinterpret_cast<const f32x4*>(partial + (long)p * n + i);
#pragma unroll
        for (int r = 0; r < 4; ++r) s[r] += v[r];
    }
    if (TR) {
        float* g = G + (i % K) * ldg + (i / K);
#pragma unroll
        for (int r = 0; r < 4; ++r) g[r * ldg] += s[r];
        return;
    }
    float* g = G + (i / K) * ldg + (i % K);
    const f32x4 o = *reinterpret_cast<const f32x4*>(g);
#pragma unroll
    for (int r = 0; r < 4; ++r) s[r] += o[r];
    *reinterpret_cast<f32x4*>(g) = s;
}

static int lin_wgrad_splits(int M, int K) {
    const int ncol = K / LIN_BM, nblk = (M + 63) / 64;
    int s = (768 + ncol - 1) / ncol;
    if (s > 16) s = 16;
    if (s > nblk) s = nblk;
    return s < 1 ? 1 : s;
}
size_t a2s_linear_wgrad_ws_bytes_impl(int M, int K) {
    if (M < 1 || K < LIN_BM || K % LIN_BM) return 0;
    const size_t nsteps = 2 * (size_t)((M + 63) / 64);
    return nsteps * 16 * 2 * 1024 + (size_t)lin_wgrad_splits(M, K) * 256 * K * sizeof(float);
}
bool a2s_linear_wgrad_ok(int M, int N, int K, long ldz, long lda, long ldg, int period, const void* dz, const void* A, const void* G) {
    return N == 256 && M >= 64 && K >= LIN_BM && K % LIN_BM == 0 && (period == 0 || (period % 4 == 0 && K % period == 0)) && lda % 4 == 0 && ldg % 4 == 0 && ldz >= 256 &&
           (((uintptr_t)dz | (uintptr_t)A | (uintptr_t)G) % 16 == 0);
}
int a2s_linear_wgrad_impl(hipStream_t st, int M, int N, int K, const float* dz, long ldz, const float* A, long lda, float* G, long ldg, const float* a_scale,
                          const float* a_shift, int period, const float* dz_absmax, const float* a_absmax, float* ws, size_t ws_bytes) {
    A2S_REQUIRE(dz && A && G && dz_absmax && ws && ((a_scale == nullptr) == (a_shift == nullptr)), "linear_wgrad: null argument");
    A2S_REQUIRE(a2s_linear_wgrad_ok(M, N, K, ldz, lda, ldg, a_scale ? period : 0, dz, A, G), "linear_wgrad: needs N = 256, K %% 128 == 0, period %% 4 == 0, 16-byte aligned rows");
    A2S_REQUIRE(((uintptr_t)ws % 16 == 0) && ws_bytes >= a2s_linear_wgrad_ws_bytes_impl(M, K), "linear_wgrad: workspace too small (%zu bytes needed)",
                a2s_linear_wgrad_ws_bytes_impl(M, K));
    const int nblk = (M + 63) / 64, nsteps = 2 * nblk, splits = lin_wgrad_splits(M, K);
    unsigned char* planes = reinterpret_cast<unsigned char*>(ws);
    float* partial = reinterpret_cast<float*>(planes + (size_t)nsteps * 16 * 2 * 1024);
    hipLaunchKernelGGL(lin_pack_dz_planes, dim3((unsigned)(((long)nsteps * 1024 + 255) / 256)), dim3(256), 0, st, dz, ldz, M, nsteps, dz_absmax, planes);
    A2S_CHECK_LAUNCH("lin_pack_dz_planes");
    LinWgradArgs a{A, lda, planes, partial, a_scale, a_shift, a_absmax, dz_absmax, M, K, a_scale ? period : K, nblk, (nblk + splits - 1) / splits, 0, 256, nullptr};
    hipLaunchKernelGGL(lin_wgrad_roles<false>, dim3(K / LIN_BM, splits), dim3(LIN_NTH), 0, st, a);
    A2S_CHECK_LAUNCH("lin_wgrad");
    const long n = 256L * K;
    hipLaunchKernelGGL(lin_wgrad_reduce<false>, dim3((unsigned)((n / 4 + 255) / 256)), dim3(256), 0, st, partial, splits, n, G, ldg, K, nullptr, nullptr);
    A2S_CHECK_LAUNCH("lin_wgrad_reduce");
    return A2S_OK;
}

#define TALLK_SLAB_BYTES (64u << 20)
int a2s_tallk_wgrad_on = 1;
int a2s_tallk_wgrad_max_splits = 0;
static long long g_tallk_launches = 0;
long a2s_tallk_wgrad_launches(void) { return (long)__atomic_load_n(&g_tallk_launches, __ATOMIC_RELAXED); }

static int tallk_splits(int M, int Np, int K) {
    const int tiles = (K / LIN_BM) * (Np / 256), nblk = (M + 63) / 64;
    int cus = a2s_device_geometry().cus;
    if (cus < 1) cus = 256;
    int s = cus / tiles;
    const size_t slab = (size_t)Np * K * sizeof(float);
    if ((size_t)s * slab > TALLK_SLAB_BYTES) s = (int)(TALLK_SLAB_BYTES / slab);
    if (s > nblk) s = nblk;
    if (a2s_tallk_wgrad_max_splits > 0 && s > a2s_tallk_wgrad_max_splits) s = a2s_tallk_wgrad_max_splits;
    return s < 1 ? 1 : s;
}
bool a2s_tallk_wgrad_ok(int M, int Np, int K, long ldp, long lda, long ldg, int transposed, const void* P, const void* A, const void* G, const void* bias) {
    return a2s_tallk_wgrad_on && M >= 64 && Np >= 256 && Np % 256 == 0 && Np <= 2048 && K >= LIN_BM && K % LIN_BM == 0 && K <= 4096 && ldp >= Np && lda >= K &&
           lda % 4 == 0 && ldg % 4 == 0 && ldg >= (transposed ? Np : K) && (((uintptr_t)P | (uintptr_t)A | (uintptr_t)G | (uintptr_t)bias) % 16 == 0);
}
size_t a2s_tallk_wgrad_ws_bytes_impl(int M, int Np, int K) {
    if (M < 1 || Np < 256 || Np % 256 || K < LIN_BM || K % LIN_BM) return 0;
    const size_t nsteps = 2 * (size_t)((M + 63) / 64), splits = (size_t)tallk_splits(M, Np, K);
    return (size_t)(Np / 256) * nsteps * 16 * 2 * 1024 + splits * Np * K * sizeof(float) + splits * K * sizeof(float);
}
int a2s_tallk_wgrad_impl(hipStream_t st, int M, int Np, int K, const float* P, long ldp, const float* A, long lda, float* G, long ldg, int transposed,
                         float* bias, const float* p_absmax, const float* a_absmax, float* ws, size_t ws_bytes) {
    A2S_REQUIRE(P && A && G && p_absmax && a_absmax && ws, "tallk_wgrad: null argument");
    A2S_REQUIRE(a2s_tallk_wgrad_ok(M, Np, K, ldp, lda, ldg, transposed, P, A, G, bias),
                "tallk_wgrad: needs M >= 64, Np %% 256 == 0, K %% 128 == 0, 16-byte aligned bases and rows (or the switch \"tallk_wgrad\" is off)");
    A2S_REQUIRE(((uintptr_t)ws % 16 == 0) && ws_bytes >= a2s_tallk_wgrad_ws_bytes_impl(M, Np, K), "tallk_wgrad: workspace too small (%zu bytes needed)",
                a2s_tallk_wgrad_ws_bytes_impl(M, Np, K));
    const int nblk = (M + 63) / 64, nsteps = 2 * nblk, splits = tallk_splits(M, Np, K), npb = Np / 256;
    const size_t plane_stride = (size_t)nsteps * 16 * 2 * 1024;
    unsigned char* planes = reinterpret_cast<unsigned char*>(ws);
    float* partial = reinterpret_cast<float*>(planes + npb * plane_stride);
    float* bias_partial = partial + (size_t)splits * Np * K;
    hipLaunchKernelGGL(lin_pack_dz_planes, dim3((unsigned)(((long)nsteps * 1024 + 255) / 256), npb), dim3(256), 0, st, P, ldp, M, nsteps, p_absmax, planes);
    A2S_CHECK_LAUNCH("lin_pack_dz_planes");
    LinWgradArgs a{A, lda, planes, partial, nullptr, nullptr, a_absmax, p_absmax, M, K, K, nblk, (nblk + splits - 1) / splits, (long)plane_stride, Np,
                   bias ? bias_partial : nullptr};
    if (bias) hipLaunchKernelGGL(lin_wgrad_roles<true>, dim3(K / LIN_BM, splits, npb), dim3(LIN_NTH), 0, st, a);
    else hipLaunchKernelGGL(lin_wgrad_roles<false>, dim3(K / LIN_BM, splits, npb), dim3(LIN_NTH), 0, st, a);
    A2S_CHECK_LAUNCH("lin_wgrad (tall-K)");
    const long n = (long)Np * K, nthreads = (n + (bias ? K : 0)) / 4;
    const dim3 rgrid((unsigned)((nthreads + 255) / 256));
    if (transposed) hipLaunchKernelGGL(lin_wgrad_reduce<true>, rgrid, dim3(256), 0, st, partial, splits, n, G, ldg, K, bias ? bias_partial : nullptr, bias);
    else hipLaunchKernelGGL(lin_wgrad_reduce<false>, rgrid, dim3(256), 0, st, partial, splits, n, G, ldg, K, bias ? bias_partial : nullptr, bias);
    A2S_CHECK_LAUNCH("lin_wgrad_reduce");
    __atomic_fetch_add(&g_tallk_launches, 1LL, __ATOMIC_RELAXED);
    return A2S_OK;
}
```

### piano_a2s_amd/engine_bwd.py

```python
import ctypes as C
import os
import threading
from collections import namedtuple

import torch

from . import hip
from .conv_bwd_plan import CHANS, ConvBwdFlags, plan_convstack_bwd
from .spec import SOS, VOCAB_SIZE


def _ptr(t, off=0):
    return C.c_void_p(t.data_ptr() + 4 * off)


_COLSUM_WS = {}


def _colsum(x, ld, out, rows, ncol, x_off=0, out_off=0, beta=1.0):
    ws = None
    if rows >= 2048:
        key = (x.device, torch.cuda.current_stream().cuda_stream, threading.get_ident())
        ws = _COLSUM_WS.get(key)
        if ws is None or ws.numel() < 1024 * ncol:
            ws = _COLSUM_WS[key] = torch.empty(1024 * max(ncol, 2048), dtype=torch.float32, device=x.device)
    hip.check(hip.lib().a2s_col_sum(hip.stream(), _ptr(x, x_off), ld, _ptr(out, out_off), rows, ncol, 1.0, beta, hip._p(ws), ws.numel() if ws is not None else 0),
              "a2s_col_sum")


def _linear_bwd(x, W, dy, G, wname, bname, dx=None, dx_beta=0.0, x_affine=None, dy_amax=None, x_bound=None):
    M, K = x.shape
    N = W.shape[0]
    sk = hip.lib().a2s_gemm_pick_splitk(N, K, M, 1)
    hip.gemm(dy, 1, N, x, K, 1, G[wname], K, N, K, M, beta=1.0, splitk=sk, b_affine=x_affine, two_term=(dy_amax, x_bound) if dy_amax is not None else None)
    if bname is not None:
        _colsum(dy, N, G[bname], M, N)
    if dx is not None:
        hip.gemm(dy, N, 1, W, K, 1, dx, dx.stride(0), M, K, N, beta=dx_beta)
    return dx


_ONES = {}


def _one(dev):
    key = torch.device(dev).index
    if key not in _ONES:
        _ONES[key] = torch.ones(1, dtype=torch.float32, device=dev)
    return _ONES[key]


def _staff_token_bwd(eng, S, G, rec, dtok):
    L = hip.lib()
    names = [f"decoder.staff_emb.{w}_{sfx}" for sfx in ("l0", "l0_reverse") for w in ("weight_ih", "weight_hh", "bias_ih", "bias_hh")]
    warr = (C.c_void_p * 8)(*[S[n].data_ptr() for n in names])
    gptrs = G.get("__staff_emb_ptrs__")
    if gptrs is None:
        gptrs = torch.tensor([G[n].data_ptr() for n in names], dtype=torch.int64, device=dtok.device)
    E, Sz = eng.cfg["note_emb_size"], eng.cfg["staff_emb_size"]
    ids = rec["ids"]
    hip.check(L.a2s_staff_emb_bwd(hip.stream(), hip._p(S["decoder.note_emb.weight"]), warr, hip._p(gptrs), hip._p(G["decoder.note_emb.weight"]),
                                  hip._p(ids) if rec["i64"] else None, None if rec["i64"] else hip._p(ids), rec["id_bstride"], hip._p(rec["lengths"]), rec["len_stride"],
                                  hip._p(dtok), dtok.stride(0), rec["col0"], hip._p(rec["hsave"]), dtok.shape[0], rec["maxlen"], E, Sz), "a2s_staff_emb_bwd")
    return gptrs


def _attn_deferred(eng, S, G, prefix, keys, enc, q_all, ds_all, attw_all, dctx_all, dK, dEnc, B, T, H, steps, active=None, groups=1):
    L = hip.lib()
    until = active["until"] if active else None
    if (2 * H == 512 and L.a2s_debug_get(b"attn_deferred_fast") > 0 and hasattr(L, "a2s_attn_denc_accum")
            and attw_all.is_contiguous() and dctx_all.is_contiguous() and dEnc.is_contiguous()):
        hip.check(L.a2s_attn_denc_accum(hip.stream(), hip._p(attw_all), hip._p(dctx_all), hip._p(dEnc), B, T, steps, 2 * H, hip._p(until), groups),
                  "a2s_attn_denc_accum")
    else:
        hip.gemm(attw_all, 1, B * T, dctx_all, B * 2 * H, 1, dEnc, 2 * H, T, 2 * H, steps * groups, beta=1.0, batch=B, bsA=T, bsB=2 * H, bsC=T * 2 * H,
                 two_term=(_one(enc.device), hip.absmax(dctx_all)) if dctx_all.is_contiguous() else None)
    nblk = L.a2s_attn_dk_blocks(B, T)
    dvp = torch.empty((nblk, H), dtype=torch.float32, device=enc.device)
    hip.check(L.a2s_attn_dk_accum(hip.stream(), hip._p(keys), hip._p(q_all), hip._p(ds_all), hip._p(S[prefix + ".v.weight"]), hip._p(dK),
                                  hip._p(dvp), B, T, steps, H, hip._p(until), groups), "a2s_attn_dk_accum")
    _colsum(dvp, H, G[prefix + ".v.weight"], nblk, H)


def _note_decoder_bwd(eng, S, G, sv, keys, enc, dprobs_bar, probs_bar, dK, dEnc, n_clips, T, deferred=None, enc_amax=None, late=None, defer_launch=False):
    L = hip.lib()
    groups = sv.get("groups", 1)
    B = groups * n_clips
    cfg = eng.cfg
    H, E, V = cfg["hidden_size"], cfg["note_emb_size"], VOCAB_SIZE
    H2, ldx = 2 * H, E + 2 * H
    n, prefix, dev = sv["steps"], sv["prefix"], enc.device
    R = n * B
    dlog = torch.empty((n, B, V), dtype=torch.float32, device=dev)
    hip.check(L.a2s_log_softmax_bwd_rows(hip.stream(), hip._p(dprobs_bar), hip._p(probs_bar), probs_bar.stride(0), n, hip._p(dlog), R, V, B, 1),
              "a2s_log_softmax_bwd_rows")
    o2d, dlog2d = sv["o"].view(R, 2 * H2), dlog.view(R, V)
    do_all = torch.empty((n, B, 2 * H2), dtype=torch.float32, device=dev)
    Wo = S[prefix + ".out.weight"]
    dlog_amax = hip.absmax(dlog) if enc_amax is not None else None
    hip.gemm(dlog2d, V, 1, Wo, 2 * H2, 1, do_all.view(R, 2 * H2), 2 * H2, R, 2 * H2, V,
             two_term=(dlog_amax, hip.absmax(Wo)) if enc_amax is not None else None)
    dgi_all = torch.empty((n, B, 3 * H2), dtype=torch.float32, device=dev)
    dgh_all = torch.empty((n, B, 3 * H2), dtype=torch.float32, device=dev)
    dq_all = torch.empty((n, B, H), dtype=torch.float32, device=dev)
    ds_all = torch.empty((n, B, T), dtype=torch.float32, device=dev)
    dctx_all = torch.empty((n, B, H2), dtype=torch.float32, device=dev)
    dx = torch.empty((n, B, ldx), dtype=torch.float32, device=dev)
    dh = torch.empty((2, B, H2), dtype=torch.float32, device=dev)
    a = hip.NoteDecBwdArgs()
    for name, t in (("attn_w", S[prefix + ".attn.attn.weight"]), ("attn_v", S[prefix + ".attn.v.weight"]), ("w_ih", S[prefix + ".gru.weight_ih_l0"]),
                    ("w_hh", S[prefix + ".gru.weight_hh_l0"]), ("keys", keys), ("enc", enc), ("h", sv["h"]), ("x", sv["x"]), ("q", sv["q"]),
                    ("gates", sv["gates"]), ("attw", sv["attw"]), ("do_all", do_all), ("dgi_all", dgi_all), ("dgh_all", dgh_all),
                    ("dq_all", dq_all), ("ds_all", ds_all), ("dctx_all", dctx_all), ("dx", dx), ("dh", dh), ("attn_ws", sv["attn_ws"]), ("gemm_ws", sv["gemm_ws"])):
        setattr(a, name, t.data_ptr() if t is not None else None)
    a.gemm_ws_bytes = sv["gemm_ws"].numel() * 4 if sv["gemm_ws"] is not None else 0
    if sv.get("step_ws") is not None:
        a.step_ws, a.step_ws_floats = sv["step_ws"].data_ptr(), sv["step_ws"].numel()
    hip.set_row_plan(a, sv.get("active"))
    a.R, a.T, a.H, a.E, a.steps = B, T, H, E, n
    a.persist_ws, a.persist_ws_bytes, a.w_ih_full = None, 0, None
    persist_ws = None
    if sv.get("persist_ws") is not None:
        nb_ws = L.a2s_note_decoder_bwd_persist_ws_bytes(n_clips)
        if nb_ws:
            persist_ws = torch.empty(nb_ws, dtype=torch.uint8, device=dev)
            a.persist_ws, a.persist_ws_bytes = persist_ws.data_ptr(), nb_ws
    if not defer_launch:
        hip.check(L.a2s_note_decoder_bwd(hip.stream(), C.byref(a)), "a2s_note_decoder_bwd")
    def deferred_work(part="all"):
        if part == "attn":
            _attn_deferred(eng, S, G, prefix + ".attn", keys, enc, sv["q"], ds_all, sv["attw"], dctx_all, dK, dEnc, n_clips, T, H, n, sv.get("active"), groups)
            return
        one = _one(dev)
        xb = torch.maximum(hip.absmax(S[prefix + ".embedding.weight"]), enc_amax) if enc_amax is not None else None
        ob = torch.maximum(one, enc_amax) if enc_amax is not None else None
        am = (lambda t: hip.absmax(t)) if enc_amax is not None else (lambda t: None)
        x2d, h2d = sv["x"][:n].view(R, ldx), sv["h"][:n].view(R, H2)
        live = sv["active"].get("live_idx") if (sv.get("active") and sv["active"].get("live_steps") == n) else None
        dlog_w, o_w, dgi_w, dgh_w, dq_w, Rw = dlog2d, o2d, dgi_all.view(R, 3 * H2), dgh_all.view(R, 3 * H2), dq_all.view(R, H), R
        if live is not None and live.numel() < 0.8 * R:
            Rw = live.numel()
            if Rw == 0:
                return
            sel = lambda t2d: t2d.index_select(0, live)
            dlog_w, o_w, dgi_w, dgh_w, dq_w, x2d, h2d = sel(dlog_w), sel(o_w), sel(dgi_w), sel(dgh_w), sel(dq_w), sel(x2d), sel(h2d)
        else:
            live = None
        _linear_bwd(o_w, Wo, dlog_w, G, prefix + ".out.weight", prefix + ".out.bias", dy_amax=dlog_amax, x_bound=ob)
        _linear_bwd(x2d, S[prefix + ".gru.weight_ih_l0"], dgi_w, G, prefix + ".gru.weight_ih_l0", prefix + ".gru.bias_ih_l0",
                    dy_amax=am(dgi_w), x_bound=xb)
        _linear_bwd(h2d, S[prefix + ".gru.weight_hh_l0"], dgh_w, G, prefix + ".gru.weight_hh_l0", prefix + ".gru.bias_hh_l0",
                    dy_amax=am(dgh_w), x_bound=one)
        Gw = G[prefix + ".attn.attn.weight"]
        sk = L.a2s_gemm_pick_splitk(H, H2, Rw, 1)
        hip.gemm(dq_w, 1, H, h2d, H2, 1, Gw, 4 * H, H, H2, Rw, beta=1.0, splitk=sk, two_term=(hip.absmax(dq_w), one) if enc_amax is not None else None)
        _colsum(dq_w, H, G[prefix + ".attn.attn.bias"], Rw, H)
        if part == "all":
            _attn_deferred(eng, S, G, prefix + ".attn", keys, enc, sv["q"], ds_all, sv["attw"], dctx_all, dK, dEnc, n_clips, T, H, n, sv.get("active"), groups)
        tok = torch.full((n, B), SOS, dtype=torch.int32, device=dev)
        if n > 1:
            prev = sv["ids"][:, :n - 1].t()
# ... 292 lines not shown
        n_conv = next(off for k, off in zip(names, offs) if not k.startswith("convstack."))
        if grad_ready is not None:
            if defer:
                with torch.cuda.stream(_weight_grad_stream(dev)):
                    grad_ready(self.flat_full, n_conv, total + 1)
            else:
                grad_ready(self.flat_full, n_conv, total + 1)
        if getattr(eng, "conv_unperm", None) is not None:
            d_conv = d_conv.reshape(B, T, -1).index_select(0, eng.conv_unperm)
        _convstack_bwd(eng, S, G, sv["conv"], d_conv, B, T, F)
        if defer:
            torch.cuda.current_stream().wait_stream(_weight_grad_stream(dev))
        if grad_ready is not None:
            grad_ready(flat, 0, n_conv)
        G[None] = flat
        G["__loss_gate__"] = self.flat_full[total:]
        eng._keep_alive = self.keep_alive
        return G




def backward(eng, S, grad_outputs, grad_ready=None, loss_total=None):
    from .engine import group_views, run_clip_groups
    sv = eng.saved
    assert sv["training"], "backward needs a forward run with training=True (batch statistics / saved activations)"
    dev = sv["enc_out"].device
    clip_groups = sv.get("clip_groups") or [(0, sv["shape"][0])]
    ctx = Backward(eng, S, sv["shape"], dev, clip_groups, sv.get("concurrent"), sv.get("bar_major"))
    dts, dkey, dup, dlo = [g.contiguous() for g in grad_outputs]

    def group(gidx):
        b0, b1 = clip_groups[gidx]
        if ctx.bar_major:
            dup_g, dlo_g = group_views(dup, clip_groups, gidx), group_views(dlo, clip_groups, gidx)
        else:
            dup_g, dlo_g = dup[b0:b1], dlo[b0:b1]
        ctx.decoder_group(gidx, sv["groups"][gidx], dts[b0:b1], dkey[b0:b1], dup_g, dlo_g)

    run_clip_groups(dev, [lambda gi=gi: group(gi) for gi in range(len(clip_groups))])
    if loss_total is not None:
        ctx.flat_full[ctx.total:].copy_(loss_total.reshape(1))
    return ctx.finish(grad_ready)


_DEFERRED_STREAMS = {}


def _deferred_streams(dev, group=0):
    idx = torch.device(dev).index if torch.device(dev).index is not None else torch.cuda.current_device()
    key = (idx, group)
    if key not in _DEFERRED_STREAMS:
        _DEFERRED_STREAMS[key] = (torch.cuda.Stream(device=idx), torch.cuda.Stream(device=idx))
    return _DEFERRED_STREAMS[key]



def _weight_grad_stream(dev):
    from .engine import group_stream
    return group_stream(dev, 1)


def _encoder_bwd(eng, S, G, es, dEnc, d_hidden, B, T, wait_weight_grads=True):
    L = hip.lib()
    H = eng.cfg["hidden_size"]
    dev = dEnc.device
    W = S["encoder.fc.weight"]
    dpre = torch.empty_like(d_hidden)
    hip.check(L.a2s_ew_act_bwd(hip.stream(), hip._p(d_hidden), hip._p(es["hidden"]), hip._p(dpre), dpre.numel(), 2), "tanh bwd")
    dhn = []
    for l in (0, 1):
        for half, hfin in enumerate((es["finals"][2 * l], es["finals"][2 * l + 1])):
            d = torch.empty((B, H), device=dev)
            hip.gemm(dpre, 2 * H, 1, W, 2 * H, 1, d, H, B, H, H, a_off=l * H, b_off=half * H)
            hip.gemm(dpre, 1, 2 * H, hfin, H, 1, G["encoder.fc.weight"], 2 * H, H, H, B, beta=1.0, a_off=l * H, c_off=half * H)
            dhn.append(d)
        _colsum(dpre, 2 * H, G["encoder.fc.bias"], B, H, x_off=l * H)
    gws = [hip.gemm_workspace(B, dev), hip.gemm_workspace(B, dev)]
    two_term = True
    in_amax = hip.absmax(es["layers"][0]["in"]) if two_term else None
    dout = dEnc
    for layer in (1, 0):
        ls = es["layers"][layer]
        inp = ls["in"]
        I = inp.shape[1]
        out = ls["out"]
        dX = torch.empty((B * T, I), device=dev)
        from .engine import encoder_streams, fork_on_streams
        streams = encoder_streams(dev, B)

        def direction(d, sfx):
            dgi = torch.empty((B, T, 3 * H), device=dev)
            dghs = torch.empty((B, T, 3 * H), device=dev)
            dgh_first, dhbuf, dgh_tmp = torch.empty((B, 3 * H), device=dev), torch.empty((2, B, H), device=dev), torch.empty((B, 3 * H), device=dev)
            ranges, valid = torch.empty(2, device=dev), C.c_int(0)
            if two_term and L.a2s_debug_get(b"tallk_wgrad") > 0:
                hip.check(L.a2s_gru_seq_bwd_ranged(hip.stream(), _ptr(dout, d * H), T * 2 * H, 2 * H, _ptr(out, d * H), T * 2 * H, 2 * H, hip._p(ls["dirs"][d]["gates"]),
                                                   hip._p(S[f"encoder.gru.weight_hh_{sfx}"]), hip._p(dhn[2 * layer + d]), hip._p(dgi), hip._p(dghs), hip._p(dgh_first),
                                                   hip._p(dhbuf), hip._p(dgh_tmp), B, T, H, d, hip._p(gws[d]), gws[d].numel() * 4, hip._p(ranges), C.byref(valid)),
                          "a2s_gru_seq_bwd_ranged")
            else:
                hip.check(L.a2s_gru_seq_bwd(hip.stream(), _ptr(dout, d * H), T * 2 * H, 2 * H, _ptr(out, d * H), T * 2 * H, 2 * H, hip._p(ls["dirs"][d]["gates"]),
                                            hip._p(S[f"encoder.gru.weight_hh_{sfx}"]), hip._p(dhn[2 * layer + d]), hip._p(dgi), hip._p(dghs), hip._p(dgh_first),
                                            hip._p(dhbuf), hip._p(dgh_tmp), B, T, H, d, hip._p(gws[d]), gws[d].numel() * 4), "a2s_gru_seq_bwd")
            return (dgi, dghs, dgh_first, dhbuf, dgh_tmp, ranges if valid.value else None)

        res = fork_on_streams(dev, streams, [lambda d=d, sfx=sfx: direction(d, sfx) for d, sfx in enumerate((f"l{layer}", f"l{layer}_reverse"))])()
        dgi_amax = []
        for d, sfx in enumerate((f"l{layer}", f"l{layer}_reverse")):
            dgi2 = res[d][0].view(B * T, 3 * H)
            Wih = S[f"encoder.gru.weight_ih_{sfx}"]
            ranges = res[d][5]
            tt = (ranges[0:1] if ranges is not None else hip.absmax(dgi2), hip.absmax(Wih)) if two_term else None
            dgi_amax.append(tt[0] if tt else None)
            if L.a2s_debug_get(b"gemm_bf16x3") > 0:
                hip.gemm(dgi2, 3 * H, 1, Wih.t().contiguous(), 1, 3 * H, dX, I, B * T, I, 3 * H, beta=0.0 if d == 0 else 1.0, two_term=tt)
            else:
                hip.gemm(dgi2, 3 * H, 1, Wih, I, 1, dX, I, B * T, I, 3 * H, beta=0.0 if d == 0 else 1.0, two_term=tt)
        wg = _weight_grad_stream(dev)
        ev = torch.cuda.Event()
        ev.record()
        wg.wait_event(ev)
        for d, sfx in enumerate((f"l{layer}", f"l{layer}_reverse")):
            dgi, dghs, dgh_first, ranges = res[d][0], res[d][1], res[d][2], res[d][5]
            for t in (dgi, dghs, dgh_first, dgi_amax[d], in_amax, ranges):
                if t is not None:
                    t.record_stream(wg)
            with torch.cuda.stream(wg):
                dgi2, dghs2 = dgi.view(B * T, 3 * H), dghs.view(B * T, 3 * H)
                x_bound = ((in_amax if layer == 0 else hip.one(dev)) if two_term else None)
                if not hip.tallk_wgrad(inp, 0, I, dgi2, 0, 3 * H, G[f"encoder.gru.weight_ih_{sfx}"], 0, I, B * T, I, 3 * H, x_bound, dgi_amax[d],
                                       transposed=True, bias=G[f"encoder.gru.bias_ih_{sfx}"]):
                    _linear_bwd(inp, S[f"encoder.gru.weight_ih_{sfx}"], dgi2, G, f"encoder.gru.weight_ih_{sfx}", f"encoder.gru.bias_ih_{sfx}",
                                dy_amax=dgi_amax[d], x_bound=x_bound)
                dghs_amax = (ranges[1:2] if ranges is not None else hip.absmax(dghs2)) if two_term else None
                if not hip.tallk_wgrad(out, d * H, 2 * H, dghs2, 0, 3 * H, G[f"encoder.gru.weight_hh_{sfx}"], 0, H, B * T, H, 3 * H,
                                       hip.one(dev) if two_term else None, dghs_amax, transposed=True, bias=G[f"encoder.gru.bias_hh_{sfx}"]):
                    sk = L.a2s_gemm_pick_splitk(3 * H, H, B * T, 1)
                    hip.gemm(dghs2, 1, 3 * H, out, 2 * H, 1, G[f"encoder.gru.weight_hh_{sfx}"], H, 3 * H, H, B * T, beta=1.0, splitk=sk, b_off=d * H,
                             two_term=(dghs_amax, hip.one(dev)) if two_term else None)
                    _colsum(dghs2, 3 * H, G[f"encoder.gru.bias_hh_{sfx}"], B * T, 3 * H)
                _colsum(dgh_first, 3 * H, G[f"encoder.gru.bias_hh_{sfx}"], B, 3 * H)
        dout = dX.view(B, T, I)
    if wait_weight_grads:
        torch.cuda.current_stream().wait_stream(_weight_grad_stream(dev))
    return dout


_FUSE_BN_APPLY = False
_FUSE_BN_APPLY_L1 = True
_DGRAD_BNSTATS = True
_SYNC_FUSED = True
_LIN_WGRAD_AT = "before"
_FUSE_BN_ROWS = os.environ.get("A2S_FUSE_BN_ROWS", "1") != "0"
GradIn = namedtuple("GradIn", "g partial amax", defaults=(None, None))


def _bn_bwd(source, eng, G, name, gin, x, bn, dims, mask=None, dx=None, amax=None):
    dgamma, dbeta = G[name + ".weight"], G[name + ".bias"]
    if source in ("own", "partial"):
        return hip.bn_bwd(gin.g, x, bn, mask, dgamma, dbeta, dx, dims, amax, gin.partial if source == "partial" else None)
    import torch.distributed as dist
    return hip.bn_bwd_sync(gin.g, x, bn, mask, dgamma, dbeta, dims, eng.bn_counts[name], dist.all_reduce, gin.partial if source == "sync_partial" else None)


def _convstack_bwd(eng, S, G, cs, d_out, B, T, F):
    if cs["a4"] is not None:
        raise ValueError("the Linear's input is re-formed from y4 on the fly: a materialised a4 has no backward path")
    L, dev, Cf, rows = hip.lib(), d_out.device, eng.cfg["conv_feature_size"], B * T
    flags = ConvBwdFlags(_FUSE_BN_ROWS, _DGRAD_BNSTATS, _SYNC_FUSED, _FUSE_BN_APPLY, _FUSE_BN_APPLY_L1, _LIN_WGRAD_AT)
    lin, layers = plan_convstack_bwd(flags, eng.sync_bn, rows, F, hip.LINEAR_KERNELS, bool(L.a2s_linear_dgrad_eligible(rows, 40 * F, Cf, F)),
                                     {c: bool(L.a2s_conv3x3_wgrad_bn_ranged_eligible(F, *c)) for c in CHANS[1:]})
    scalar = lambda: torch.zeros(1, dtype=torch.float32, device=dev)
    dz, dz_amax = d_out.reshape(rows, Cf).contiguous(), scalar()
    _bn_bwd(lin.stats, eng, G, "convstack.out_bn", GradIn(dz), cs["z"], cs["out_bn"], (rows, Cf, 1), cs["drop"], dz, dz_amax)
    if lin.absmax_after:
        hip.absmax(dz, dz_amax)
    Wout, y4, bn4 = S["convstack.out.weight"], cs["y"][3].view(rows, 40 * F), cs["bn"][3]
    da = torch.empty_like(y4)

    def lin_wgrad():
        if not hip.linear_wgrad(dz, y4, (bn4[2], bn4[3], F), dz_amax, cs["abound"][3], G["convstack.out.weight"]):
            _linear_bwd(y4, Wout, dz, G, "convstack.out.weight", None, x_affine=(bn4[2], bn4[3], F), dy_amax=dz_amax, x_bound=cs["abound"][3])
    def lin_wgrad_beside():
        wg_stream, ev = _weight_grad_stream(dev), torch.cuda.Event()
        ev.record()
        wg_stream.wait_event(ev)
        with torch.cuda.stream(wg_stream):
            lin_wgrad()
    if lin.wgrad_at in ("before", "beside"):
        (lin_wgrad if lin.wgrad_at == "before" else lin_wgrad_beside)()
    gin = GradIn(da.view(B, T, 40, F))
    if lin.dgrad == "gemm":
        hip.gemm(dz, Cf, 1, Wout, 40 * F, 1, da, 40 * F, rows, 40 * F, Cf)
    else:
        w_amax = cs["w_out_amax"] if cs.get("w_out_amax") is not None else hip.absmax(Wout)
        gin = GradIn(gin.g, *hip.linear_dgrad_bnstats(dz, Wout, da, y4, bn4, F, dz_amax, w_amax, lin.dgrad == "own"))
    for lp in layers:
        i, ci, co, g = lp.i, lp.ci, lp.co, gin.g
        y, bn_i, dW = cs["y"][i - 1], cs["bn"][i - 1], G[f"convstack.conv{i}.weight"]
        x_in, in_bn, in_bound = (cs["y"][i - 2], cs["bn"][i - 2], cs["abound"][i - 2]) if i > 1 else (cs["x0"], None, None)
        ws = torch.empty(L.a2s_conv3x3_wgrad_workspace_bytes(ci, co) // 4, dtype=torch.float32, device=dev)
        dy_amax = scalar() if lp.dy_range else None
        if lp.lin_wgrad:
            lin_wgrad_beside()
        bn_args = (lp.stats, eng, G, f"convstack.bn{i}", gin, y, bn_i, (rows, co, F))
        dy = g
        if lp.form == "rows":
            hip.conv3x3_wgrad_bn(g, y, bn_i, _bn_bwd(*bn_args), None, x_in, in_bn, dW, ws, ranged=(gin.amax, cs["yabs"][i - 1], dy_amax, in_bound))
        elif lp.form == "apply":
            _bn_bwd(*bn_args, dx=g, amax=dy_amax)
            if lp.absmax_after:
                hip.absmax(g, dy_amax)
            hip.conv3x3_wgrad(g, x_in.view(B, T, ci, F), in_bn[2] if in_bn else None, in_bn[3] if in_bn else None, dW, ws, dy_amax, in_bound)
        else:
            dy = torch.empty_like(g) if i > 1 else None
            hip.conv3x3_wgrad_bn(g, y, bn_i, _bn_bwd(*bn_args), dy, x_in, in_bn, dW, ws)
        if lp.dgrad == "none":
            break
        gprev, cws = torch.empty((B, T, ci, F), dtype=torch.float32, device=dev), hip.conv_workspace(co, dev)
        below = nblk = out_amax = None
        if lp.dgrad == "bnstats":
            nblk = L.a2s_conv3x3_stat_blocks(B, T, F, co)
            below = (x_in, in_bn, torch.empty((nblk, ci, 2), dtype=torch.float32, device=dev))
            out_amax = torch.empty(ci, dtype=torch.float32, device=dev) if lp.out_range else None
        hip.conv3x3_dgrad(dy, S[f"convstack.conv{i}.weight"], gprev, cws, below, dy_amax if lp.dgrad_range else None, out_amax)
        gin = GradIn(gprev, (below[2], nblk) if below else None, out_amax)
    if lin.join_side:
        torch.cuda.current_stream().wait_stream(_weight_grad_stream(dev))
```

### piano_a2s_amd/hip.py

```python
import ctypes as C
import os
import threading

import torch

from .abi import PROTOTYPES, STRUCTS, A2SError
from .build import LIB

LIB = os.environ.get("A2S_LIB", LIB)

NoteDecArgs, NoteDecBwdArgs, BeamArgs, AlignArgs = (STRUCTS[n] for n in ("a2s_note_dec_args", "a2s_note_dec_bwd_args", "a2s_beam_args", "a2s_align_args"))
_lib = None


def set_row_plan(a, active):
    active = active or {}
    for field, key in (("clip_order", "order"), ("clip_rank", "rank"), ("row_until", "until"), ("row_list", "row_list")):
        setattr(a, field, active[key].data_ptr() if active.get(key) is not None else None)
    for field, key in (("n_active", "n_active"), ("m_active", "m_active"), ("n_rows_active", "n_rows_active")):
        host = active.get(key) if (key != "n_rows_active" or active.get("row_list") is not None) else None
        setattr(a, field, C.cast(host, C.c_void_p).value if host is not None else None)
    a.n_clips = active.get("n_clips", 0)


# ... 607 lines not shown
    return out


def note_match_launches():
    return int(lib().a2s_note_match_launches())


def align_buffers(R, max_steps, T, device):
    t = dict(attw_step=torch.zeros((R, T), dtype=torch.float32, device=device),
             peak=torch.full((R, max_steps), -1, dtype=torch.int32, device=device),
             weight=torch.zeros((R, max_steps), dtype=torch.float32, device=device),
             centroid=torch.full((R, max_steps), -1.0, dtype=torch.float32, device=device))
    g = AlignArgs()
    for name in ("attw_step", "peak", "weight", "centroid"):
        setattr(g, name, t[name].data_ptr())
    g.out_stride = max_steps
    g.next_state, g.n_states, g.row_state = None, 0, None
    return g, t


def check(rc, what):
    if rc != 0:
        raise A2SError(f"{what} failed ({rc}): {lib().a2s_last_error().decode()}")


def f32(x):
    return C.c_float(float(x))


def gemm(A, sAm, sAk, B, sBk, sBn, Cout, ldc, M, N, K, alpha=1.0, beta=0.0, bias=None, act=0,
         batch=1, bsA=0, bsB=0, bsC=0, splitk=1, a_off=0, b_off=0, c_off=0, a_affine=None, b_affine=None, two_term=None):
    L = lib()
    ws, ws_bytes = None, 0
    if splitk > 1:
        ws_bytes = L.a2s_gemm_workspace_bytes(M, N, batch, splitk)
        ws = torch.empty(ws_bytes // 4, dtype=torch.float32, device=Cout.device)
    pa = C.c_void_p(A.data_ptr() + 4 * a_off)
    pb = C.c_void_p(B.data_ptr() + 4 * b_off)
    pc = C.c_void_p(Cout.data_ptr() + 4 * c_off)
    if a_affine is None and b_affine is None and two_term is None:
        check(L.a2s_gemm_f32(stream(), M, N, K, alpha, pa, sAm, sAk, pb, sBk, sBn, beta, pc, ldc, _p(bias), act, batch, bsA, bsB, bsC, splitk, _p(ws), ws_bytes),
              "a2s_gemm_f32")
        return
    asc, ash, ap = a_affine if a_affine is not None else (None, None, 0)
    bsc, bsh, bp = b_affine if b_affine is not None else (None, None, 0)
    if two_term is not None:
        check(L.a2s_gemm_f32_affine_scaled(stream(), M, N, K, alpha, pa, sAm, sAk, pb, sBk, sBn, beta, pc, ldc, _p(bias), act, batch, bsA, bsB, bsC, splitk, _p(ws),
                                           ws_bytes, _p(asc), _p(ash), ap, _p(bsc), _p(bsh), bp, _p(two_term[0]), _p(two_term[1])), "a2s_gemm_f32_affine_scaled")
        return
    check(L.a2s_gemm_f32_affine(stream(), M, N, K, alpha, pa, sAm, sAk, pb, sBk, sBn, beta, pc, ldc, _p(bias), act, batch, bsA, bsB, bsC, splitk, _p(ws), ws_bytes,
                                _p(asc), _p(ash), ap, _p(bsc), _p(bsh), bp), "a2s_gemm_f32_affine")


_ONES = {}


def one(device):
    key = torch.device(device).index
    if key not in _ONES:
        _ONES[key] = torch.ones(1, dtype=torch.float32, device=device)
    return _ONES[key]


def absmax(x, out=None):
    if out is None:
        out = torch.empty(1, dtype=torch.float32, device=x.device)
    check(lib().a2s_absmax(stream(), _p(x), x.numel(), _p(out)), "a2s_absmax")
    return out


def linear(x2d, weight, bias=None, act=0, out=None, beta=0.0, x_affine=None, two_term=None):
    M, K = x2d.shape
    N = weight.shape[0]
    if out is None:
        out = torch.empty((M, N), dtype=torch.float32, device=x2d.device)
    gemm(x2d, x2d.stride(0), x2d.stride(1), weight, weight.stride(1), weight.stride(0), out, out.stride(0), M, N, K,
         bias=bias, act=act, beta=beta, a_affine=x_affine, two_term=two_term)
    return out


def conv3x3_forward(x, w, y, scale, shift, partial, cws, in_absmax=None, out_absmax=None):
    B, T, Cin, F = x.shape
    check(lib().a2s_conv3x3_ranged(stream(), _p(x), _p(w), _p(y), _p(scale), _p(shift), _p(in_absmax), _p(partial), _p(out_absmax),
                                   B, T, F, Cin, y.shape[2], _p(cws)), "a2s_conv3x3_ranged")


def conv3x3_dgrad_for_test(dy, w, yl):
    (B, T, Cout, F), Cin, dev = dy.shape, w.shape[1], dy.device
    dx = torch.full((B, T, Cin, F), float("nan"), device=dev)
    part = torch.zeros(lib().a2s_conv3x3_stat_blocks(B, T, F, Cout), Cin, 2, device=dev)
    zeros, ones = torch.zeros(Cin, device=dev), torch.ones(Cin, device=dev)
    conv3x3_dgrad(dy, w, dx, conv_workspace(Cout, dev), (yl, (zeros, ones, ones, zeros), part), absmax(dy))
    torch.cuda.synchronize()
    return dx


def act_bound(scale, shift, x_absmax):
    out = torch.empty(1, dtype=torch.float32, device=scale.device)
    check(lib().a2s_act_bound(stream(), _p(scale), _p(shift), _p(x_absmax), scale.numel(), _p(out)), "a2s_act_bound")
    return out


def conv3x3_wgrad(dy, x, scale, shift, dW, ws, dy_absmax, act_absmax):
    B, T, Cout, F = dy.shape
    Cin = x.shape[2]
    check(lib().a2s_conv3x3_wgrad_ranged(stream(), _p(dy), _p(x), _p(scale), _p(shift), _p(dW), _p(ws), ws.numel() * 4, B, T, F, Cin, Cout, _p(dy_absmax),
                                         _p(act_absmax)), "a2s_conv3x3_wgrad_ranged")


def conv3x3_wgrad_for_test(dy, x, scale, shift):
    L = lib()
    B, T, Cout, F = dy.shape
    Cin = x.shape[2]
    dev = dy.device
    dW = torch.zeros(Cout, Cin, 3, 3, device=dev)
    ws = torch.empty(L.a2s_conv3x3_wgrad_workspace_bytes(Cin, Cout) // 4, device=dev)
    bound = act_bound(scale, shift, x.abs().amax(dim=(0, 1, 3)).contiguous())
    conv3x3_wgrad(dy, x, scale, shift, dW, ws, absmax(dy), bound)
    torch.cuda.synchronize()
    return dW


def linear_forward(x2d, weight, x_affine, x_bound, w_absmax, out=None):
    M, K = x2d.shape
    N = weight.shape[0]
    L = lib()
    period = x_affine[2]
    if (LINEAR_KERNELS and x2d.is_contiguous() and weight.is_contiguous() and x_bound is not None
            and L.a2s_linear_fwd_eligible(M, N, K, period)):
        if out is None:
            out = torch.empty((M, N), dtype=torch.float32, device=x2d.device)
        nb = L.a2s_linear_dgrad_ws_bytes(N, K)
        ws = torch.empty(nb // 4, dtype=torch.float32, device=x2d.device)
        check(L.a2s_linear_fwd(stream(), M, N, K, _p(x2d), K, _p(weight), _p(out), N, _p(x_affine[0]), _p(x_affine[1]), period, _p(x_bound), _p(w_absmax), _p(ws), nb),
              "a2s_linear_fwd")
        return out
    return linear(x2d, weight, out=out, x_affine=x_affine, two_term=(x_bound, w_absmax))


def linear_wgrad(dz, x2d, x_affine, dz_absmax, x_bound, G):
    M, K = x2d.shape
    N = dz.shape[1]
    L = lib()
    if (not LINEAR_KERNELS or not (x2d.is_contiguous() and dz.is_contiguous() and G.is_contiguous()) or dz_absmax is None
            or x_bound is None or not L.a2s_linear_wgrad_eligible(M, N, K, x_affine[2])):
        return False
    nb = L.a2s_linear_wgrad_ws_bytes(M, K)
    ws = torch.empty(nb // 4, dtype=torch.float32, device=x2d.device)
    check(L.a2s_linear_wgrad(stream(), M, N, K, _p(dz), N, _p(x2d), K, _p(G), K, _p(x_affine[0]), _p(x_affine[1]), x_affine[2], _p(dz_absmax), _p(x_bound), _p(ws), nb),
          "a2s_linear_wgrad")
    return True


def _f32(like, *shape):
    return torch.empty(shape, dtype=torch.float32, device=like.device)


def bn_bwd(g, x, bn, mask, dgamma, dbeta, dx, dims, amax, partial=None):
    c12 = _f32(g, 2 * dims[1])
    if partial is None:
        part = _f32(g, lib().a2s_bn_bwd_partial_floats(*dims))
        check(lib().a2s_bn_bwd_amax(stream(), _p(g), _p(x), *map(_p, bn), _p(mask), 1.0 / 0.8, _p(dgamma), _p(dbeta), _p(dx), _p(part), _p(c12), *dims, _p(amax)),
              "a2s_bn_bwd")
    else:
        check(lib().a2s_bn_bwd_from_partial_amax(stream(), _p(g), _p(x), *map(_p, bn), _p(dgamma), _p(dbeta), _p(dx), _p(partial[0]), partial[1], _p(c12), *dims,
                                                 _p(amax)), "a2s_bn_bwd_from_partial")
    return c12


def bn_bwd_sync(g, x, bn, mask, dgamma, dbeta, dims, count, all_reduce, partial=None):
    L, local, c12 = lib(), _f32(g, 2 * dims[1]), _f32(g, 2 * dims[1])
    if partial is None:
        part = _f32(g, L.a2s_bn_bwd_partial_floats(*dims))
        check(L.a2s_bn_bwd_stats(stream(), _p(g), _p(x), *map(_p, bn), _p(mask), 1.0 / 0.8, _p(part), _p(local), *dims), "a2s_bn_bwd_stats")
    else:
        check(L.a2s_bn_bwd_sums_from_partial(stream(), _p(partial[0]), partial[1], dims[1], _p(local)), "a2s_bn_bwd_sums_from_partial")
    glob = local.clone()
    all_reduce(glob)
    if partial is None:
        check(L.a2s_bn_bwd_apply(stream(), _p(g), _p(x), *map(_p, bn), _p(mask), 1.0 / 0.8, _p(local), _p(glob), count, _p(dgamma), _p(dbeta), _p(g), _p(c12), *dims),
              "a2s_bn_bwd_apply")
    else:
        check(L.a2s_bn_bwd_c12_from_sums(stream(), _p(local), _p(glob), count, _p(dgamma), _p(dbeta), _p(c12), dims[1]), "a2s_bn_bwd_c12_from_sums")
    return c12


def conv3x3_wgrad_bn(g, y, bn, c12, dy, x, in_bn, dW, ws, ranged=None):
    B, T, _, F = g.shape
    sc, sh = in_bn[2:] if in_bn else (None, None)
    tail = _p(x), _p(sc), _p(sh), _p(dW), _p(ws), ws.numel() * 4, B, T, F, dW.shape[1], dW.shape[0]
    if ranged is None:
        return check(lib().a2s_conv3x3_wgrad_bn(stream(), _p(g), _p(y), *map(_p, bn), _p(c12), _p(dy), *tail), "a2s_conv3x3_wgrad_bn")
    g_absmax, y_absmax, dy_absmax, act_absmax = ranged
    check(lib().a2s_conv3x3_wgrad_bn_ranged(stream(), _p(g), _p(y), *map(_p, bn), _p(c12), _p(g_absmax), g_absmax.numel(), _p(y_absmax), _p(g), _p(dy_absmax), *tail,
                                            _p(act_absmax)), "a2s_conv3x3_wgrad_bn_ranged")


def conv3x3_dgrad(dy, w, dx, cws, below=None, dy_absmax=None, out_absmax=None):
    B, T, _, F = dy.shape
    if below is None:
        return check(lib().a2s_conv3x3(stream(), _p(dy), _p(w), _p(dx), None, None, None, B, T, F, w.shape[0], w.shape[1], 1, _p(cws)), "a2s_conv3x3 dgrad")
    check(lib().a2s_conv3x3_dgrad_bnstats_ranged(stream(), _p(dy), _p(w), _p(dx), _p(below[0]), *map(_p, below[1]), _p(below[2]), B, T, F, w.shape[0], w.shape[1],
                                                 _p(cws), _p(dy_absmax), _p(out_absmax)), "a2s_conv3x3_dgrad_bnstats")


def linear_dgrad_bnstats(dz, W, da, y, bn, F, dz_absmax, w_absmax, own):
    L, (rows, Cf), K = lib(), dz.shape, W.shape[1]
    nblk = L.a2s_linear_dgrad_blocks(rows) if own else L.a2s_gemm_bnstats_blocks(rows, F)
    part = _f32(dz, nblk, K // F, 2)
    if own:
        nb = L.a2s_linear_dgrad_ws_bytes(K, Cf)
        Wt, ws, amax = W.t().contiguous(), _f32(dz, nb // 4), torch.zeros(1, dtype=torch.float32, device=dz.device)
        check(L.a2s_linear_dgrad_bnstats(stream(), rows, K, Cf, _p(dz), Cf, _p(Wt), _p(da), K, _p(y), *map(_p, bn), F, _p(part), _p(dz_absmax), _p(w_absmax), _p(ws), nb,
                                         _p(amax)), "a2s_linear_dgrad_bnstats")
        return (part, nblk), amax
    wb, s_bk, s_bn = (W.t().contiguous(), 1, Cf) if L.a2s_debug_get(b"gemm_bf16x3") > 0 else (W, K, 1)
    check(L.a2s_gemm_f32_bnstats_scaled(stream(), rows, K, Cf, _p(dz), Cf, 1, _p(wb), s_bk, s_bn, _p(da), K, _p(y), *map(_p, bn), F, _p(part), _p(dz_absmax), _p(w_absmax)),
          "a2s_gemm_f32_bnstats_scaled")
    return (part, nblk), None


_TALLK_WS = {}


def tallk_wgrad(P, p_off, ldp, A, a_off, lda, G, g_off, ldg, M, Np, K, p_absmax, a_absmax, transposed=False, bias=None):
    L = lib()
    if not hasattr(L, "a2s_tallk_wgrad_eligible"):
        return False
    pp, pa, pg = P.data_ptr() + 4 * p_off, A.data_ptr() + 4 * a_off, G.data_ptr() + 4 * g_off
    if (p_absmax is None or a_absmax is None or (pp | pa | pg | (bias.data_ptr() if bias is not None else 0)) % 16
            or not L.a2s_tallk_wgrad_eligible(M, Np, K, ldp, lda, ldg, int(transposed))):
        return False
    nb = L.a2s_tallk_wgrad_ws_bytes(M, Np, K)
    key = (A.device, torch.cuda.current_stream().cuda_stream, threading.get_ident())
    ws = _TALLK_WS.get(key)
    if ws is None or ws.numel() * 4 < nb:
        ws = _TALLK_WS[key] = torch.empty((nb + 3) // 4, dtype=torch.float32, device=A.device)
    check(L.a2s_tallk_wgrad(stream(), M, Np, K, C.c_void_p(pp), ldp, C.c_void_p(pa), lda, C.c_void_p(pg), ldg, int(transposed), _p(bias), _p(p_absmax), _p(a_absmax),
                            _p(ws), ws.numel() * 4), "a2s_tallk_wgrad")
    return True


def linear_forward_for_test(x, w, aff):
    period = aff[2]
    xmax = x.view(x.shape[0], -1, period).abs().amax(dim=(0, 2)).contiguous()
    return linear_forward(x, w, aff, act_bound(aff[0], aff[1], xmax), absmax(w))
```

Measured before the change: 638.3.

## Reuse Linear wgrad's ReLU mask and W·G dot to derive dgrad BN stats

The Linear weight-gradient kernel now writes a packed ReLU mask bitfield and computes per-channel W·G dot products. The data-gradient kernel can then use the mask instead of reloading y4 and the BN affine parameters. The second BN statistic is recovered algebraically in a small fixup kernel from wdotg and the masked sum. A guard kernel falls back to the original path at runtime when the channel scale or shift makes the algebra unsafe. This removes the y4 reads from the dgrad kernel but adds several small launches, fp64 reductions and a mask buffer.

```diff
diff --git a/include/a2s.h b/include/a2s.h
--- a/include/a2s.h
+++ b/include/a2s.h
@@ -48,6 +48,16 @@
 size_t a2s_linear_dgrad_ws_bytes(int N, int K);
 int a2s_linear_dgrad_blocks(int M);
 int a2s_linear_dgrad_eligible(int M, int N, int K, int period);
+int a2s_linear_wgrad_mask(void* stream, int M, int N, int K, const float* dz, long ldz, const float* y, long lda, float* G, long ldg, const float* scale,
+                          const float* shift, int period, const float* dz_absmax, const float* y_absmax, float* workspace, size_t workspace_bytes,
+                          const float* W, long ldw, uint8_t* relu_mask, size_t relu_mask_bytes, double* wdotg);
+int a2s_linear_dgrad_maskstats(void* stream, int M, int N, int K, const float* dz, long lda, const float* Wt, float* da, long ldc, const float* y,
+                               const float* mean, const float* invstd, const float* scale, const float* shift, int period, float* partial,
+                               const float* dz_absmax, const float* w_absmax, float* workspace, size_t workspace_bytes, float* da_absmax_out,
+                               uint8_t* relu_mask, size_t relu_mask_bytes, const double* wdotg);
+int a2s_linear_maskstats_eligible(int M, int N, int K, int period);
+size_t a2s_linear_relu_mask_bytes(int M, int K);
+size_t a2s_linear_relu_mask_flag_offset(int M, int K);
 int a2s_absmax(void* stream, const float* x, long n, float* out);
 int a2s_gemm_bnstats_blocks(int M, int period);
 size_t a2s_gemm_workspace_bytes(int M, int N, int batch, int splitk);
diff --git a/piano_a2s_amd/conv_bwd_plan.py b/piano_a2s_amd/conv_bwd_plan.py
--- a/piano_a2s_amd/conv_bwd_plan.py
+++ b/piano_a2s_amd/conv_bwd_plan.py
@@ -76,3 +76,7 @@
                                 i > 1 and stats and dy_range and not flags.fuse_bn_apply, out_range))
         partial, amax = stats, out_range
     return linear, tuple(layers)
+
+
+def linear_maskstats(enabled, sync_bn, linear, wgrad_operands, library_eligible):
+    return bool(enabled and linear.dgrad == "own" and linear.wgrad_at == "before" and not sync_bn and wgrad_operands and library_eligible())
diff --git a/piano_a2s_amd/csrc/a2s_api.hip b/piano_a2s_amd/csrc/a2s_api.hip
--- a/piano_a2s_amd/csrc/a2s_api.hip
+++ b/piano_a2s_amd/csrc/a2s_api.hip
@@ -71,6 +71,22 @@
 int a2s_linear_dgrad_eligible(int M, int N, int K, int period) {
     return a2s_linear_dgrad_ok(M, N, K, 4, 1, K, 4, period, nullptr, nullptr, nullptr, nullptr) ? 1 : 0;
 }
+int a2s_linear_wgrad_mask(void* stream, int M, int N, int K, const float* dz, long ldz, const float* y, long lda, float* G, long ldg, const float* scale,
+                          const float* shift, int period, const float* dz_absmax, const float* y_absmax, float* workspace, size_t workspace_bytes,
+                          const float* W, long ldw, uint8_t* relu_mask, size_t relu_mask_bytes, double* wdotg) {
+    return a2s_linear_wgrad_mask_impl(ST, M, N, K, dz, ldz, y, lda, G, ldg, scale, shift, period, dz_absmax, y_absmax, workspace, workspace_bytes, W, ldw,
+                                      relu_mask, relu_mask_bytes, wdotg);
+}
+int a2s_linear_dgrad_maskstats(void* stream, int M, int N, int K, const float* dz, long lda, const float* Wt, float* da, long ldc, const float* y,
+                               const float* mean, const float* invstd, const float* scale, const float* shift, int period, float* partial,
+                               const float* dz_absmax, const float* w_absmax, float* workspace, size_t workspace_bytes, float* da_absmax_out,
+                               uint8_t* relu_mask, size_t relu_mask_bytes, const double* wdotg) {
+    return a2s_linear_dgrad_maskstats_impl(ST, M, N, K, dz, lda, Wt, da, ldc, y, mean, invstd, scale, shift, period, partial, dz_absmax, w_absmax,
+                                           workspace, workspace_bytes, da_absmax_out, relu_mask, relu_mask_bytes, wdotg);
+}
+int a2s_linear_maskstats_eligible(int M, int N, int K, int period) { return a2s_linear_maskstats_ok(M, N, K, period) ? 1 : 0; }
+size_t a2s_linear_relu_mask_bytes(int M, int K) { return a2s_linear_relu_mask_bytes_impl(M, K); }
+size_t a2s_linear_relu_mask_flag_offset(int M, int K) { return a2s_linear_relu_mask_flag_offset_impl(M, K); }
 int a2s_gemm_f32_bnstats(void* stream, int M, int N, int K, const float* A, long sAm, long sAk, const float* B, long sBk, long sBn, float* C, long ldc,
                          const float* y, const float* mean, const float* invstd, const float* scale, const float* shift, int period, float* partial) {
     return a2s_gemm_affine_impl(ST, M, N, K, 1.f, A, sAm, sAk, B, sBk, sBn, 0.f, C, ldc, nullptr, 0, 1, 0, 0, 0, 1, nullptr, 0,
@@ -87,6 +103,7 @@
     if (id >= 0) { a2s_switch_store(id, value); return A2S_OK; }
     if (!strcmp(key, "attn_deferred_fast")) { a2s_attn_deferred_fast = value ? 1 : 0; return A2S_OK; }
     if (!strcmp(key, "tallk_wgrad")) { a2s_tallk_wgrad_on = value ? 1 : 0; return A2S_OK; }
+    if (!strcmp(key, "lin_maskstats")) { a2s_lin_maskstats_on = value ? 1 : 0; return A2S_OK; }
     if (!strcmp(key, "tallk_wgrad_max_splits")) { a2s_tallk_wgrad_max_splits = value > 0 ? value : 0; return A2S_OK; }
     if (!strcmp(key, "gemm_tile")) { a2s_gemm_debug_tile_impl(value); return A2S_OK; }
     snprintf(a2s_err_msg, sizeof(a2s_err_msg), "a2s_debug_set: unknown key %s", key);
@@ -108,6 +125,8 @@
     if (!strcmp(key, "attn_pair_bwd_launches")) return (int)a2s_attn_pair_bwd_launches();
     if (!strcmp(key, "attn_deferred_fast")) return a2s_attn_deferred_fast;
     if (!strcmp(key, "tallk_wgrad")) return a2s_tallk_wgrad_on;
+    if (!strcmp(key, "lin_maskstats")) return a2s_lin_maskstats_on;
+    if (!strcmp(key, "lin_maskstats_launches")) return (int)a2s_lin_maskstats_launches();
     if (!strcmp(key, "tallk_wgrad_max_splits")) return a2s_tallk_wgrad_max_splits;
     if (!strcmp(key, "tallk_wgrad_launches")) return (int)a2s_tallk_wgrad_launches();
     if (!strcmp(key, "attn_dk_ahead_launches")) return (int)a2s_attn_dk_ahead_launches();
diff --git a/piano_a2s_amd/csrc/a2s_internal.h b/piano_a2s_amd/csrc/a2s_internal.h
--- a/piano_a2s_amd/csrc/a2s_internal.h
+++ b/piano_a2s_amd/csrc/a2s_internal.h
@@ -39,6 +39,17 @@
 bool a2s_linear_wgrad_ok(int M, int N, int K, long ldz, long lda, long ldg, int period, const void* dz, const void* A, const void* G);
 int a2s_linear_wgrad_impl(hipStream_t st, int M, int N, int K, const float* dz, long ldz, const float* A, long lda, float* G, long ldg, const float* a_scale,
     const float* a_shift, int period, const float* dz_absmax, const float* a_absmax, float* ws, size_t ws_bytes);
+extern int a2s_lin_maskstats_on;
+long a2s_lin_maskstats_launches(void);
+bool a2s_linear_maskstats_ok(int M, int N, int K, int period);
+size_t a2s_linear_relu_mask_bytes_impl(int M, int K);
+size_t a2s_linear_relu_mask_flag_offset_impl(int M, int K);
+int a2s_linear_wgrad_mask_impl(hipStream_t st, int M, int N, int K, const float* dz, long ldz, const float* A, long lda, float* G, long ldg, const float* a_scale,
+    const float* a_shift, int period, const float* dz_absmax, const float* a_absmax, float* ws, size_t ws_bytes, const float* W, long ldw,
+    unsigned char* mask, size_t mask_bytes, double* wdotg);
+int a2s_linear_dgrad_maskstats_impl(hipStream_t st, int M, int N, int K, const float* A, long lda, const float* Wt, float* C, long ldc, const float* ep_y,
+    const float* mean, const float* invstd, const float* scale, const float* shift, int period, float* partial, const float* a_absmax,
+    const float* b_absmax, float* ws, size_t ws_bytes, float* c_absmax_out, unsigned char* mask, size_t mask_bytes, const double* wdotg);
 extern int a2s_tallk_wgrad_on;
 extern int a2s_tallk_wgrad_max_splits;
 long a2s_tallk_wgrad_launches(void);
diff --git a/piano_a2s_amd/csrc/a2s_linear.hip b/piano_a2s_amd/csrc/a2s_linear.hip
--- a/piano_a2s_amd/csrc/a2s_linear.hip
+++ b/piano_a2s_amd/csrc/a2s_linear.hip
@@ -18,7 +18,14 @@
     const float* a_absmax; const float* b_absmax;
     int M, N, period, channels;
     float* c_absmax_out;
+    const int* flag;
+    const unsigned char* mask;
 };
+
+#define LIN_MASK_TAIL 256
+#define LIN_WD_PARTS 16
+#define LIN_WD_MAX_CHANNELS 512
+static inline size_t lin_mask_bits_bytes(int M, int K) { return (size_t)((M + LIN_BM - 1) / LIN_BM) * (size_t)(K / 32) * 512; }
 
 __global__ __launch_bounds__(256) void lin_pack_planes_k(const float* __restrict__ W, long ld, int N, int K, const float* __restrict__ absmax,
                                                          unsigned char* __restrict__ out) {
@@ -41,8 +48,10 @@
     *reinterpret_cast<lu32x4*>(o + 64 * 16) = lo;
 }
 
-__global__ __launch_bounds__(LIN_NTH) void lin_dgrad_bnstats(LinDgradArgs a) {
+template <bool MASK>
+__device__ __forceinline__ void lin_dgrad_body(const LinDgradArgs& a) {
     __shared__ __attribute__((aligned(16))) unsigned char lds[LIN_LDS];
+    if (a.flag && (*a.flag != 0) != MASK) return;
     const int tid = threadIdx.x, lane = tid & 63, wave = tid >> 6, lr = lane & 15, lk = lane >> 4;
     const int m0 = blockIdx.x * LIN_BM;
     const int ka = pow2_scale_exp(*a.a_absmax, 12), kb = pow2_scale_exp(*a.b_absmax, 12);
@@ -110,8 +119,15 @@
 #endif
             }
         };
-#pragma unroll
-        for (int mt = 0; mt < 3; ++mt) load_y(mt);
+        lu32x4 mq[2];
+        if (MASK) {
+            const unsigned char* mp = a.mask + ((long)blockIdx.x * (a.N >> 5) + (n0 >> 5)) * 512 + (unsigned)((lr >> 2) * 4 + lk) * 32u;
+            mq[0] = *reinterpret_cast<const lu32x4*>(mp);
+            mq[1] = *reinterpret_cast<const lu32x4*>(mp + 16);
+        } else {
+#pragma unroll
+            for (int mt = 0; mt < 3; ++mt) load_y(mt);
+        }
         f32x4 acc[8][2];
 #pragma unroll
         for (int mt = 0; mt < 8; ++mt)
@@ -142,11 +158,14 @@
             }
         }
         if (n0 + 256 < a.N) { load_b(n0 + 256, 0, bf[0]); load_b(n0 + 256, 1, bf[1]); }
-#pragma unroll
-        for (int mt = 3; mt < 8; ++mt) load_y(mt);
+        if (!MASK) {
+#pragma unroll
+            for (int mt = 3; mt < 8; ++mt) load_y(mt);
+        }
         const int c = n0 / a.period;
         if (c != cur_c) { flush(); s1 = 0.f; s2 = 0.f; cur_c = c; }
-        const float mean = a.mean[c], invstd = a.invstd[c], sc = a.scale[c], sh = a.shift[c];
+        float mean = 0.f, invstd = 0.f, sc = 0.f, sh = 0.f;
+        if (!MASK) { mean = a.mean[c]; invstd = a.invstd[c]; sc = a.scale[c]; sh = a.shift[c]; }
 #pragma unroll
         for (int mt = 0; mt < 8; ++mt) {
             const int m = m0 + mt * 16 + lr;
@@ -160,6 +179,12 @@
                 if (v[0] == 123.456f)
 #endif
                 *reinterpret_cast<f32x4*>(reinterpret_cast<char*>(a.C + (long)(m0 + mt * 16) * a.ldc + n0 + nt * 16) + lane_off) = v;
+                if (MASK) {
+                    const unsigned bits = mq[nt][mt >> 1] >> (16 * (mt & 1) + 4 * (lr & 3));
+#pragma unroll
+                    for (int r = 0; r < 4; ++r) s1 += ((bits >> r) & 1u) ? v[r] : 0.f;
+                    continue;
+                }
 #pragma unroll
                 for (int r = 0; r < 4; ++r) {
                     const float gm = (fmaf(yq[mt][nt][r], sc, sh) > 0.f) ? v[r] : 0.f;
@@ -172,6 +197,38 @@
     if (a.c_absmax_out) {
         const float m = wave_max(vmax);
         if (lane == 0 && m > 0.f) atomicMax(reinterpret_cast<unsigned*>(a.c_absmax_out), __float_as_uint(m));
+    }
+}
+__global__ __launch_bounds__(LIN_NTH) void lin_dgrad_bnstats(LinDgradArgs a) { lin_dgrad_body<false>(a); }
+__global__ __launch_bounds__(LIN_NTH) void lin_dgrad_maskstats(LinDgradArgs a) { lin_dgrad_body<true>(a); }
+
+__global__ __launch_bounds__(256) void lin_maskstats_guard(const float* __restrict__ mean, const float* __restrict__ invstd, const float* __restrict__ scale,
+                                                           const float* __restrict__ shift, int channels, int* __restrict__ flag) {
+    int ok = 1;
+    for (int c = threadIdx.x; c < channels; c += 256) {
+        const float sc = scale[c], beta = fmaf(mean[c], sc, shift[c]);
+        ok &= (isfinite(sc) && sc != 0.f && fabsf(beta) * invstd[c] <= 16.f * fabsf(sc)) ? 1 : 0;
+    }
+    ok = __syncthreads_and(ok);
+    if (threadIdx.x == 0) *flag = ok ? 1 : 0;
+}
+__global__ __launch_bounds__(256) void lin_maskstats_fixup(float* __restrict__ partial, int nblocks, int channels, const double* __restrict__ wdotg,
+                                                           const float* __restrict__ mean, const float* __restrict__ invstd, const float* __restrict__ scale,
+                                                           const float* __restrict__ shift, const int* __restrict__ flag) {
+    if (*flag == 0) return;
+    const int c = blockIdx.x;
+    __shared__ double r1[256];
+    double s1 = 0.0;
+    for (int i = threadIdx.x; i < nblocks; i += 256) s1 += (double)partial[((long)i * channels + c) * 2];
+    r1[threadIdx.x] = s1;
+    __syncthreads();
+    for (int o = 128; o > 0; o >>= 1) {
+        if (threadIdx.x < o) r1[threadIdx.x] += r1[threadIdx.x + o];
+        __syncthreads();
+    }
+    if (threadIdx.x == 0) {
+        const double sc = scale[c], beta = (double)shift[c] + (double)mean[c] * sc;
+        partial[(long)c * 2 + 1] = (float)((double)invstd[c] / sc * (wdotg[c] - beta * r1[0]));
     }
 }
 
@@ -197,9 +254,52 @@
     unsigned char* planes = reinterpret_cast<unsigned char*>(ws);
     hipLaunchKernelGGL(lin_pack_planes_k, dim3((unsigned)(((long)N * (K / 8) + 255) / 256)), dim3(256), 0, st, Wt, (long)K, N, K, b_absmax, planes);
     A2S_CHECK_LAUNCH("lin_pack_planes_k");
-    LinDgradArgs a{A, lda, planes, C, ldc, ep_y, mean, invstd, scale, shift, partial, a_absmax, b_absmax, M, N, period, channels, c_absmax_out};
+    LinDgradArgs a{A, lda, planes, C, ldc, ep_y, mean, invstd, scale, shift, partial, a_absmax, b_absmax, M, N, period, channels, c_absmax_out, nullptr, nullptr};
     hipLaunchKernelGGL(lin_dgrad_bnstats, dim3((M + LIN_BM - 1) / LIN_BM), dim3(LIN_NTH), 0, st, a);
     A2S_CHECK_LAUNCH("lin_dgrad_bnstats");
+    return A2S_OK;
+}
+
+int a2s_lin_maskstats_on = 1;
+static long long g_maskstats_launches = 0;
+long a2s_lin_maskstats_launches(void) { return (long)__atomic_load_n(&g_maskstats_launches, __ATOMIC_RELAXED); }
+size_t a2s_linear_relu_mask_bytes_impl(int M, int K) { return (M > 0 && K > 0 && K % 32 == 0) ? lin_mask_bits_bytes(M, K) + LIN_MASK_TAIL : 0; }
+size_t a2s_linear_relu_mask_flag_offset_impl(int M, int K) { return (M > 0 && K > 0 && K % 32 == 0) ? lin_mask_bits_bytes(M, K) : 0; }
+bool a2s_linear_maskstats_ok(int M, int N, int K, int period) {
+    return a2s_lin_maskstats_on && a2s_linear_dgrad_ok(M, N, K, 4, 1, K, 4, period, nullptr, nullptr, nullptr, nullptr) &&
+           a2s_linear_wgrad_ok(M, K, N, 256, 4, 4, period, nullptr, nullptr, nullptr) && N / period <= LIN_WD_MAX_CHANNELS;
+}
+
+int a2s_linear_dgrad_maskstats_impl(hipStream_t st, int M, int N, int K, const float* A, long lda, const float* Wt, float* C, long ldc, const float* ep_y,
+                                    const float* mean, const float* invstd, const float* scale, const float* shift, int period, float* partial,
+                                    const float* a_absmax, const float* b_absmax, float* ws, size_t ws_bytes, float* c_absmax_out, unsigned char* mask,
+                                    size_t mask_bytes, const double* wdotg) {
+    A2S_REQUIRE(A && Wt && C && ep_y && mean && invstd && scale && shift && partial && a_absmax && b_absmax && ws && mask && wdotg,
+                "linear_dgrad_maskstats: null argument");
+    A2S_REQUIRE(a2s_linear_maskstats_ok(M, N, K, period) && a2s_linear_dgrad_ok(M, N, K, lda, 1, K, ldc, period, A, Wt, C, ep_y),
+                "linear_dgrad_maskstats: needs the shapes of linear_dgrad_bnstats and of linear_wgrad_mask (N %% 128 == 0, period %% 32 == 0) and the switch \"lin_maskstats\"");
+    A2S_REQUIRE(((uintptr_t)ws % 16 == 0) && ws_bytes >= a2s_linear_dgrad_ws_bytes_impl(N, K), "linear_dgrad_maskstats: workspace too small (%zu bytes needed)",
+                a2s_linear_dgrad_ws_bytes_impl(N, K));
+    A2S_REQUIRE(((uintptr_t)mask % 16 == 0) && mask_bytes >= a2s_linear_relu_mask_bytes_impl(M, N), "linear_dgrad_maskstats: mask buffer too small (%zu bytes needed)",
+                a2s_linear_relu_mask_bytes_impl(M, N));
+    const int channels = N / period, nblk = a2s_linear_dgrad_blocks_impl(M);
+    hipError_t e = hipMemsetAsync(partial, 0, sizeof(float) * 2 * (size_t)nblk * channels, st);
+    if (e != hipSuccess) A2S_FAIL(A2S_ERR_HIP, "linear_dgrad_maskstats memset: %s", hipGetErrorString(e));
+    unsigned char* planes = reinterpret_cast<unsigned char*>(ws);
+    int* flag = reinterpret_cast<int*>(mask + lin_mask_bits_bytes(M, N));
+    hipLaunchKernelGGL(lin_maskstats_guard, dim3(1), dim3(256), 0, st, mean, invstd, scale, shift, channels, flag);
+    A2S_CHECK_LAUNCH("lin_maskstats_guard");
+    hipLaunchKernelGGL(lin_pack_planes_k, dim3((unsigned)(((long)N * (K / 8) + 255) / 256)), dim3(256), 0, st, Wt, (long)K, N, K, b_absmax, planes);
+    A2S_CHECK_LAUNCH("lin_pack_planes_k");
+    LinDgradArgs a{A, lda, planes, C, ldc, ep_y, mean, invstd, scale, shift, partial, a_absmax, b_absmax, M, N, period, channels, c_absmax_out, flag, mask};
+    const dim3 grid((M + LIN_BM - 1) / LIN_BM);
+    hipLaunchKernelGGL(lin_dgrad_maskstats, grid, dim3(LIN_NTH), 0, st, a);
+    A2S_CHECK_LAUNCH("lin_dgrad_maskstats");
+    hipLaunchKernelGGL(lin_dgrad_bnstats, grid, dim3(LIN_NTH), 0, st, a);
+    A2S_CHECK_LAUNCH("lin_dgrad_bnstats (guarded)");
+    hipLaunchKernelGGL(lin_maskstats_fixup, dim3(channels), dim3(256), 0, st, partial, nblk, channels, wdotg, mean, invstd, scale, shift, flag);
+    A2S_CHECK_LAUNCH("lin_maskstats_fixup");
+    __atomic_fetch_add(&g_maskstats_launches, 1LL, __ATOMIC_RELAXED);
     return A2S_OK;
 }
 
@@ -370,6 +470,7 @@
     int M, K, period, nblk, blk_per_split;
     long plane_stride; int np;
     float* bias_partial;
+    unsigned char* mask;
 };
 
 __global__ __launch_bounds__(256) void lin_pack_dz_planes(const float* __restrict__ dz, long ld, int M, int nsteps, const float* __restrict__ absmax,
@@ -395,7 +496,7 @@
     *reinterpret_cast<lu32x4*>(o + 64 * 16) = lo;
 }
 
-template <bool BIAS>
+template <bool BIAS, bool MASK>
 __global__ __launch_bounds__(LIN_NTH) void lin_wgrad_roles(LinWgradArgs a) {
     __shared__ __attribute__((aligned(16))) unsigned char lds[LF_NS * LF_STAGE];
     const int tid = threadIdx.x, lane = tid & 63, lr = lane & 15, lk = lane >> 4;
@@ -408,11 +509,12 @@
     if (wave >= 4) {
         const int st_ = tid - 256;
         const int rq = st_ & 15, cq0 = st_ >> 4;
-        float sc[2], sh[2];
+        float sc[2], sh[2], sc0[2] = {0.f, 0.f}, sh0[2] = {0.f, 0.f};
 #pragma unroll
         for (int u = 0; u < 2; ++u) {
             const int ch = affine ? (k0 + 4 * (cq0 + 16 * u)) / a.period : 0;
             sc[u] = affine ? a.a_scale[ch] * psa : psa; sh[u] = affine ? a.a_shift[ch] * psa : 0.f;
+            if (MASK) { sc0[u] = a.a_scale[ch]; sh0[u] = a.a_shift[ch]; }
         }
         const float floor_ = affine ? 0.f : -INFINITY;
         f32x4 ar[2][8];
@@ -437,6 +539,19 @@
                     for (int j = 0; j < 4; ++j)
 #pragma unroll
                         for (int c = 0; c < 4; ++c) bs[u][c] += r[4 * u + j][c];
+            }
+            if (MASK) {
+                unsigned char* mp = a.mask + ((long)(blk >> 1) * (a.K >> 5) + (k0 >> 5) + (cq0 >> 3)) * 512 +
+                                    (unsigned)(((rq & 3) * 4 + (cq0 & 3)) * 32 + ((cq0 >> 2) & 1) * 16 + (4 * (blk & 1) + (rq >> 2)) * 2);
+#pragma unroll
+                for (int u = 0; u < 2; ++u) {
+                    unsigned bits = 0;
+#pragma unroll
+                    for (int j = 0; j < 4; ++j)
+#pragma unroll
+                        for (int c = 0; c < 4; ++c) bits |= (fmaf(r[4 * u + j][c], sc0[u], sh0[u]) > 0.f ? 1u : 0u) << (4 * j + c);
+                    *reinterpret_cast<unsigned short*>(mp + u * 2 * 512) = (unsigned short)bits;
+                }
             }
 #pragma unroll
             for (int u = 0; u < 2; ++u)
@@ -622,12 +737,75 @@
     float* partial = reinterpret_cast<float*>(planes + (size_t)nsteps * 16 * 2 * 1024);
     hipLaunchKernelGGL(lin_pack_dz_planes, dim3((unsigned)(((long)nsteps * 1024 + 255) / 256)), dim3(256), 0, st, dz, ldz, M, nsteps, dz_absmax, planes);
     A2S_CHECK_LAUNCH("lin_pack_dz_planes");
-    LinWgradArgs a{A, lda, planes, partial, a_scale, a_shift, a_absmax, dz_absmax, M, K, a_scale ? period : K, nblk, (nblk + splits - 1) / splits, 0, 256, nullptr};
-    hipLaunchKernelGGL(lin_wgrad_roles<false>, dim3(K / LIN_BM, splits), dim3(LIN_NTH), 0, st, a);
+    LinWgradArgs a{A, lda, planes, partial, a_scale, a_shift, a_absmax, dz_absmax, M, K, a_scale ? period : K, nblk, (nblk + splits - 1) / splits, 0, 256, nullptr, nullptr};
+    hipLaunchKernelGGL((lin_wgrad_roles<false, false>), dim3(K / LIN_BM, splits), dim3(LIN_NTH), 0, st, a);
     A2S_CHECK_LAUNCH("lin_wgrad");
     const long n = 256L * K;
     hipLaunchKernelGGL(lin_wgrad_reduce<false>, dim3((unsigned)((n / 4 + 255) / 256)), dim3(256), 0, st, partial, splits, n, G, ldg, K, nullptr, nullptr);
     A2S_CHECK_LAUNCH("lin_wgrad_reduce");
+    return A2S_OK;
+}
+
+__global__ __launch_bounds__(256) void lin_wdotg(const float* __restrict__ slabs, int splits, long n, const float* __restrict__ W, long ldw, int K, int period,
+                                                 double* __restrict__ parts) {
+    const int c = blockIdx.x, part = blockIdx.y, pq = period >> 2, rows = 256 / LIN_WD_PARTS;
+    __shared__ double red[256];
+    double s = 0.0;
+    for (int e = threadIdx.x; e < rows * pq; e += 256) {
+        const int row = part * rows + e / pq, k = c * period + (e % pq) * 4;
+        const long i = (long)row * K + k;
+        f32x4 g = *reinterpret_cast<const f32x4*>(slabs + i);
+        for (int p = 1; p < splits; ++p) {
+            const f32x4 v = *reinterpret_cast<const f32x4*>(slabs + (long)p * n + i);
+#pragma unroll
+            for (int r = 0; r < 4; ++r) g[r] += v[r];
+        }
+        const f32x4 w = *reinterpret_cast<const f32x4*>(W + (long)row * ldw + k);
+#pragma unroll
+        for (int r = 0; r < 4; ++r) s += (double)w[r] * (double)g[r];
+    }
+    red[threadIdx.x] = s;
+    __syncthreads();
+    for (int o = 128; o > 0; o >>= 1) {
+        if (threadIdx.x < o) red[threadIdx.x] += red[threadIdx.x + o];
+        __syncthreads();
+    }
+    if (threadIdx.x == 0) parts[c * LIN_WD_PARTS + part] = red[0];
+}
+__global__ __launch_bounds__(256) void lin_wdotg_sum(const double* __restrict__ parts, int channels, double* __restrict__ out) {
+    const int c = blockIdx.x * 256 + threadIdx.x;
+    if (c >= channels) return;
+    double s = 0.0;
+    for (int p = 0; p < LIN_WD_PARTS; ++p) s += parts[c * LIN_WD_PARTS + p];
+    out[c] = s;
+}
+
+int a2s_linear_wgrad_mask_impl(hipStream_t st, int M, int N, int K, const float* dz, long ldz, const float* A, long lda, float* G, long ldg, const float* a_scale,
+                               const float* a_shift, int period, const float* dz_absmax, const float* a_absmax, float* ws, size_t ws_bytes, const float* W, long ldw,
+                               unsigned char* mask, size_t mask_bytes, double* wdotg) {
+    A2S_REQUIRE(dz && A && G && dz_absmax && ws && a_scale && a_shift && W && mask && wdotg, "linear_wgrad_mask: null argument");
+    A2S_REQUIRE(a2s_linear_wgrad_ok(M, N, K, ldz, lda, ldg, period, dz, A, G) && a2s_linear_maskstats_ok(M, K, N, period) && ldw >= K && ldw % 4 == 0 &&
+                    ((uintptr_t)W | (uintptr_t)mask | (uintptr_t)wdotg) % 16 == 0,
+                "linear_wgrad_mask: needs the shapes of linear_wgrad and of linear_dgrad_bnstats (M >= 128, period %% 32 == 0), 16-byte aligned rows and the switch \"lin_maskstats\"");
+    A2S_REQUIRE(((uintptr_t)ws % 16 == 0) && ws_bytes >= a2s_linear_wgrad_ws_bytes_impl(M, K), "linear_wgrad_mask: workspace too small (%zu bytes needed)",
+                a2s_linear_wgrad_ws_bytes_impl(M, K));
+    A2S_REQUIRE(mask_bytes >= a2s_linear_relu_mask_bytes_impl(M, K), "linear_wgrad_mask: mask buffer too small (%zu bytes needed)", a2s_linear_relu_mask_bytes_impl(M, K));
+    const int nblk = (M + 63) / 64, nsteps = 2 * nblk, splits = lin_wgrad_splits(M, K), channels = K / period;
+    unsigned char* planes = reinterpret_cast<unsigned char*>(ws);
+    float* partial = reinterpret_cast<float*>(planes + (size_t)nsteps * 16 * 2 * 1024);
+    hipLaunchKernelGGL(lin_pack_dz_planes, dim3((unsigned)(((long)nsteps * 1024 + 255) / 256)), dim3(256), 0, st, dz, ldz, M, nsteps, dz_absmax, planes);
+    A2S_CHECK_LAUNCH("lin_pack_dz_planes");
+    LinWgradArgs a{A, lda, planes, partial, a_scale, a_shift, a_absmax, dz_absmax, M, K, period, nblk, (nblk + splits - 1) / splits, 0, 256, nullptr, mask};
+    hipLaunchKernelGGL((lin_wgrad_roles<false, true>), dim3(K / LIN_BM, splits), dim3(LIN_NTH), 0, st, a);
+    A2S_CHECK_LAUNCH("lin_wgrad (mask)");
+    const long n = 256L * K;
+    hipLaunchKernelGGL(lin_wgrad_reduce<false>, dim3((unsigned)((n / 4 + 255) / 256)), dim3(256), 0, st, partial, splits, n, G, ldg, K, nullptr, nullptr);
+    A2S_CHECK_LAUNCH("lin_wgrad_reduce");
+    double* parts = reinterpret_cast<double*>(planes);
+    hipLaunchKernelGGL(lin_wdotg, dim3(channels, LIN_WD_PARTS), dim3(256), 0, st, partial, splits, n, W, ldw, K, period, parts);
+    A2S_CHECK_LAUNCH("lin_wdotg");
+    hipLaunchKernelGGL(lin_wdotg_sum, dim3((channels + 255) / 256), dim3(256), 0, st, parts, channels, wdotg);
+    A2S_CHECK_LAUNCH("lin_wdotg_sum");
     return A2S_OK;
 }
 
@@ -672,9 +850,9 @@
     hipLaunchKernelGGL(lin_pack_dz_planes, dim3((unsigned)(((long)nsteps * 1024 + 255) / 256), npb), dim3(256), 0, st, P, ldp, M, nsteps, p_absmax, planes);
     A2S_CHECK_LAUNCH("lin_pack_dz_planes");
     LinWgradArgs a{A, lda, planes, partial, nullptr, nullptr, a_absmax, p_absmax, M, K, K, nblk, (nblk + splits - 1) / splits, (long)plane_stride, Np,
-                   bias ? bias_partial : nullptr};
-    if (bias) hipLaunchKernelGGL(lin_wgrad_roles<true>, dim3(K / LIN_BM, splits, npb), dim3(LIN_NTH), 0, st, a);
-    else hipLaunchKernelGGL(lin_wgrad_roles<false>, dim3(K / LIN_BM, splits, npb), dim3(LIN_NTH), 0, st, a);
+                   bias ? bias_partial : nullptr, nullptr};
+    if (bias) hipLaunchKernelGGL((lin_wgrad_roles<true, false>), dim3(K / LIN_BM, splits, npb), dim3(LIN_NTH), 0, st, a);
+    else hipLaunchKernelGGL((lin_wgrad_roles<false, false>), dim3(K / LIN_BM, splits, npb), dim3(LIN_NTH), 0, st, a);
     A2S_CHECK_LAUNCH("lin_wgrad (tall-K)");
     const long n = (long)Np * K, nthreads = (n + (bias ? K : 0)) / 4;
     const dim3 rgrid((unsigned)((nthreads + 255) / 256));
diff --git a/piano_a2s_amd/engine_bwd.py b/piano_a2s_amd/engine_bwd.py
--- a/piano_a2s_amd/engine_bwd.py
+++ b/piano_a2s_amd/engine_bwd.py
@@ -6,7 +6,7 @@
 import torch
 
 from . import hip
-from .conv_bwd_plan import CHANS, ConvBwdFlags, plan_convstack_bwd
+from .conv_bwd_plan import CHANS, ConvBwdFlags, linear_maskstats, plan_convstack_bwd
 from .spec import SOS, VOCAB_SIZE
 
 
@@ -605,6 +605,7 @@
 _DGRAD_BNSTATS = True
 _SYNC_FUSED = True
 _LIN_WGRAD_AT = "before"
+_LIN_MASKSTATS = True
 _FUSE_BN_ROWS = os.environ.get("A2S_FUSE_BN_ROWS", "1") != "0"
 GradIn = namedtuple("GradIn", "g partial amax", defaults=(None, None))
 
@@ -631,6 +632,8 @@
         hip.absmax(dz, dz_amax)
     Wout, y4, bn4 = S["convstack.out.weight"], cs["y"][3].view(rows, 40 * F), cs["bn"][3]
     da = torch.empty_like(y4)
+    maskstats = linear_maskstats(_LIN_MASKSTATS, eng.sync_bn, lin, cs["abound"][3] is not None, lambda: L.a2s_linear_maskstats_eligible(rows, 40 * F, Cf, F))
+    mask_wdotg = None
 
     def lin_wgrad():
         if not hip.linear_wgrad(dz, y4, (bn4[2], bn4[3], F), dz_amax, cs["abound"][3], G["convstack.out.weight"]):
@@ -641,14 +644,16 @@
         wg_stream.wait_event(ev)
         with torch.cuda.stream(wg_stream):
             lin_wgrad()
-    if lin.wgrad_at in ("before", "beside"):
+    if maskstats:
+        mask_wdotg = hip.linear_wgrad_mask(dz, y4, (bn4[2], bn4[3], F), dz_amax, cs["abound"][3], G["convstack.out.weight"], Wout)
+    elif lin.wgrad_at in ("before", "beside"):
         (lin_wgrad if lin.wgrad_at == "before" else lin_wgrad_beside)()
     gin = GradIn(da.view(B, T, 40, F))
     if lin.dgrad == "gemm":
         hip.gemm(dz, Cf, 1, Wout, 40 * F, 1, da, 40 * F, rows, 40 * F, Cf)
     else:
         w_amax = cs["w_out_amax"] if cs.get("w_out_amax") is not None else hip.absmax(Wout)
-        gin = GradIn(gin.g, *hip.linear_dgrad_bnstats(dz, Wout, da, y4, bn4, F, dz_amax, w_amax, lin.dgrad == "own"))
+        gin = GradIn(gin.g, *hip.linear_dgrad_bnstats(dz, Wout, da, y4, bn4, F, dz_amax, w_amax, lin.dgrad == "own", mask_wdotg))
     for lp in layers:
         i, ci, co, g = lp.i, lp.ci, lp.co, gin.g
         y, bn_i, dW = cs["y"][i - 1], cs["bn"][i - 1], G[f"convstack.conv{i}.weight"]
diff --git a/piano_a2s_amd/hip.py b/piano_a2s_amd/hip.py
--- a/piano_a2s_amd/hip.py
+++ b/piano_a2s_amd/hip.py
@@ -783,6 +783,37 @@
     return True
 
 
+_MASKSTATS_WS = {}
+
+
+def _maskstats_ws(device, mask_bytes, channels):
+    mask, wdotg = _MASKSTATS_WS.get(device, (None, None))
+    if mask is None or mask.numel() < mask_bytes or wdotg.numel() < channels:
+        for old in (mask, wdotg):
+            if old is not None:
+                old.zero_()
+        mask = torch.empty(max(mask_bytes, mask.numel() if mask is not None else 0), dtype=torch.uint8, device=device)
+        wdotg = torch.empty(max(channels, wdotg.numel() if wdotg is not None else 0), dtype=torch.float64, device=device)
+        _MASKSTATS_WS[device] = (mask, wdotg)
+    return mask, wdotg
+
+
+def linear_wgrad_mask(dz, x2d, x_affine, dz_absmax, x_bound, G, W):
+    M, K = x2d.shape
+    N = dz.shape[1]
+    L = lib()
+    if not (x2d.is_contiguous() and dz.is_contiguous() and G.is_contiguous() and W.is_contiguous()) or dz_absmax is None or x_bound is None:
+        raise A2SError("linear_wgrad_mask: contiguous operands, max |dz| and the activation bound are required")
+    mb = L.a2s_linear_relu_mask_bytes(M, K)
+    nb = L.a2s_linear_wgrad_ws_bytes(M, K)
+    mask, wdotg = _maskstats_ws(x2d.device, mb, K // x_affine[2])
+    mask, wdotg = mask[:mb], wdotg[:K // x_affine[2]]
+    ws = torch.empty(nb // 4, dtype=torch.float32, device=x2d.device)
+    check(L.a2s_linear_wgrad_mask(stream(), M, N, K, _p(dz), N, _p(x2d), K, _p(G), K, _p(x_affine[0]), _p(x_affine[1]), x_affine[2], _p(dz_absmax), _p(x_bound),
+                                  _p(ws), nb, _p(W), K, _p(mask), mb, _p(wdotg)), "a2s_linear_wgrad_mask")
+    return mask, wdotg
+
+
 def _f32(like, *shape):
     return torch.empty(shape, dtype=torch.float32, device=like.device)
 
@@ -835,15 +866,19 @@
                                                  _p(cws), _p(dy_absmax), _p(out_absmax)), "a2s_conv3x3_dgrad_bnstats")
 
 
-def linear_dgrad_bnstats(dz, W, da, y, bn, F, dz_absmax, w_absmax, own):
+def linear_dgrad_bnstats(dz, W, da, y, bn, F, dz_absmax, w_absmax, own, maskstats=None):
     L, (rows, Cf), K = lib(), dz.shape, W.shape[1]
     nblk = L.a2s_linear_dgrad_blocks(rows) if own else L.a2s_gemm_bnstats_blocks(rows, F)
     part = _f32(dz, nblk, K // F, 2)
     if own:
         nb = L.a2s_linear_dgrad_ws_bytes(K, Cf)
         Wt, ws, amax = W.t().contiguous(), _f32(dz, nb // 4), torch.zeros(1, dtype=torch.float32, device=dz.device)
-        check(L.a2s_linear_dgrad_bnstats(stream(), rows, K, Cf, _p(dz), Cf, _p(Wt), _p(da), K, _p(y), *map(_p, bn), F, _p(part), _p(dz_absmax), _p(w_absmax), _p(ws), nb,
-                                         _p(amax)), "a2s_linear_dgrad_bnstats")
+        args = (stream(), rows, K, Cf, _p(dz), Cf, _p(Wt), _p(da), K, _p(y), *map(_p, bn), F, _p(part), _p(dz_absmax), _p(w_absmax), _p(ws), nb, _p(amax))
+        if maskstats is not None:
+            mask, wdotg = maskstats
+            check(L.a2s_linear_dgrad_maskstats(*args, _p(mask), mask.numel(), _p(wdotg)), "a2s_linear_dgrad_maskstats")
+        else:
+            check(L.a2s_linear_dgrad_bnstats(*args), "a2s_linear_dgrad_bnstats")
         return (part, nblk), amax
     wb, s_bk, s_bn = (W.t().contiguous(), 1, Cf) if L.a2s_debug_get(b"gemm_bf16x3") > 0 else (W, K, 1)
     check(L.a2s_gemm_f32_bnstats_scaled(stream(), rows, K, Cf, _p(dz), Cf, 1, _p(wb), s_bk, s_bn, _p(da), K, _p(y), *map(_p, bn), F, _p(part), _p(dz_absmax), _p(w_absmax)),
```

Result: no change. 640.1 (median of 6 runs) (+0.3%).
